# BinomialLLC/basis_universal

Measured on AMD Instinct MI355X. Metric: encoder Mpixels/s (ETC1S frontend hot path), higher is better.
Workload: dtype u8/int32; 1 GPU; 4096x4096 synthetic RGBA (SURVEY 8d recipe, seed 1234), ETC1S -q128 comp_level 1, basisu_frontend init+compress with tiles resident in HBM; blocks=1048576, max_endpoint_clusters=2416, max_selector_clusters=2731, final_endpoint_clusters=2413, final_selector_clusters=2277, images_in_flight_per_gpu=1, parallelism=1 x one image per GPU (no collective)

## Files before the change

### basis_universal_amd/csrc/api_etc1s.cpp

```cpp
#include <atomic>
#include <cstdlib>
#include "api_internal.h"
#include "etc1s_kernels.h"
#include "mipmap_kernels.h"
#include "unique_kernels.h"
#include "bookkeeping_kernels.h"
#include "kmeans_kernels.h"
#include "host/seam_translate.h"

namespace {
constexpr uint32_t UP_PIECE_BLOCKS = 65536;
constexpr uint32_t UP_SLOTS = 8, UP_EVENTS = 64;
unsigned upload_threads() {
    static const unsigned t = [] {
        unsigned want = 4;
        if (const char* e = std::getenv("BU_UPLOAD_THREADS")) { const int v = std::atoi(e); if (v >= 1 && v <= 16) want = (unsigned)v; }
        const unsigned hw = std::thread::hardware_concurrency();
        return hw ? std::min(want, std::max(1u, hw / 2)) : 1u;
    }();
    return t;
}
}

extern "C" {

int bu_hip_set_pixel_blocks(bu_hip_context* ctx, size_t total_blocks, const bu_pixel_block* blocks) {
    if (!ctx) return 0;
    if (total_blocks > 0xFFFFFFFFull) { set_error(ctx, "too many blocks"); return 0; }
    device_guard g(ctx->device);
    BU_TRY(ctx, ctx->pixel_arena.reserve(total_blocks * sizeof(bu_pixel_block)));
    if (total_blocks) BU_TRY(ctx, h2d(ctx, ctx->pixel_arena.p, blocks, total_blocks * sizeof(bu_pixel_block)));
    BU_TRY(ctx, stream_wait(ctx, ctx->stream));
    ctx->d_pixel_blocks = ctx->pixel_arena.p;
    ctx->total_blocks = total_blocks;
    return 1;
}

int bu_hip_set_pixel_blocks_device(bu_hip_context* ctx, size_t total_blocks, const void* d_blocks) {
    if (!ctx || total_blocks > 0xFFFFFFFFull) return 0;
    ctx->d_pixel_blocks = d_blocks;
    ctx->total_blocks = total_blocks;
    return 1;
}

const void* bu_hip_get_pixel_blocks_device(const bu_hip_context* ctx, size_t* total_blocks) {
    if (!ctx) return nullptr;
    if (total_blocks) *total_blocks = ctx->total_blocks;
    return ctx->d_pixel_blocks;
}


int bu_hip_k_encode_etc1s_blocks(bu_hip_context* ctx, const void* d_px, uint32_t n, int quality, int perceptual, void* d_out) {
    if (!ctx) return 0;
    device_guard g(ctx->device);
    prof_scope ps(ctx, "encode_etc1s_blocks");
    BU_TRY(ctx, bu::launch_encode_etc1s_blocks(ctx->stream, d_px, n, quality, perceptual != 0, d_out));
    return 1;
}

int bu_hip_k_upload_and_encode_etc1s_blocks(bu_hip_context* ctx, void* d_px, const void* h_px, uint32_t n, int quality, int perceptual, void* d_out) {
    if (!ctx) return 0;
    if (!n) return 1;
    if (!d_px || !h_px || !d_out) { set_error(ctx, "upload_and_encode_etc1s_blocks: null argument"); return 0; }
    device_guard g(ctx->device);
    const uint32_t n_pieces = (n + UP_PIECE_BLOCKS - 1) / UP_PIECE_BLOCKS;
    if (ctx->wait_hook || n_pieces < 2 || !ensure_side_stream(ctx)) {
        BU_TRY(ctx, h2d(ctx, d_px, h_px, (size_t)n * 64));
        prof_scope ps(ctx, "encode_etc1s_blocks");
        BU_TRY(ctx, bu::launch_encode_etc1s_blocks(ctx->stream, d_px, n, quality, perceptual != 0, d_out));
        return 1;
    }
    while (ctx->up_events.size() < UP_EVENTS) {
        hipEvent_t e = nullptr;
        BU_TRY(ctx, hipEventCreateWithFlags(&e, hipEventDisableTiming));
        ctx->up_events.push_back(e);
    }
    bool pinned_src = false;
    {
        hipPointerAttribute_t a;
        if (hipPointerGetAttributes(&a, h_px) == hipSuccess) pinned_src = a.type == hipMemoryTypeHost;
        else (void)hipGetLastError();
    }
    const size_t piece_bytes = (size_t)UP_PIECE_BLOCKS * 64;
    if (!pinned_src && ctx->up_ring_cap < piece_bytes * UP_SLOTS) {
        if (ctx->up_ring) { (void)hipHostFree(ctx->up_ring); ctx->up_ring = nullptr; ctx->up_ring_cap = 0; }
        BU_TRY(ctx, hipHostMalloc(&ctx->up_ring, piece_bytes * UP_SLOTS, hipHostMallocDefault));
        ctx->up_ring_cap = piece_bytes * UP_SLOTS;
    }
    BU_TRY(ctx, hipEventRecord(ctx->side_fork, ctx->stream));
    BU_TRY(ctx, hipStreamWaitEvent(ctx->side_stream, ctx->side_fork, 0));
    const char* src = static_cast<const char*>(h_px);
    char* dst = static_cast<char*>(d_px);
    char* out = static_cast<char*>(d_out);
    std::vector<std::atomic<int>> ready(pinned_src ? 0 : n_pieces), issued(pinned_src ? 0 : n_pieces);
    std::atomic<int> stop{0};
    std::vector<std::thread> helpers;
    if (!pinned_src) {
        for (auto& r : ready) r.store(0, std::memory_order_relaxed);
        for (auto& r : issued) r.store(0, std::memory_order_relaxed);
        const unsigned T = std::min<unsigned>(upload_threads(), n_pieces);
        try {
            for (unsigned t = 0; t < T; t++)
                helpers.emplace_back([&, t, T] {
                    (void)hipSetDevice(ctx->device);
                    for (uint32_t i = t; i < n_pieces && !stop.load(std::memory_order_acquire); i += T) {
                        if (i >= UP_SLOTS) {
                            while (!issued[i - UP_SLOTS].load(std::memory_order_acquire)) { if (stop.load(std::memory_order_acquire)) return; std::this_thread::yield(); }
                            (void)hipEventSynchronize(ctx->up_events[(i - UP_SLOTS) % UP_EVENTS]);
                        }
                        const size_t at = (size_t)i * piece_bytes, bytes = std::min(piece_bytes, (size_t)n * 64 - at);
                        std::memcpy(static_cast<char*>(ctx->up_ring) + (size_t)(i % UP_SLOTS) * piece_bytes, src + at, bytes);
                        ready[i].store(1, std::memory_order_release);
                    }
                });
        } catch (...) {
            stop.store(1); for (auto& h : helpers) h.join();
            set_error(ctx, "upload_and_encode_etc1s_blocks: could not start the helper threads");
            return 0;
        }
    }
    hipError_t err = hipSuccess;
    {
        prof_scope ps(ctx, "upload_and_encode_etc1s_blocks");
        for (uint32_t i = 0; i < n_pieces && err == hipSuccess; i++) {
            const size_t at = (size_t)i * piece_bytes, bytes = std::min(piece_bytes, (size_t)n * 64 - at);
            const uint32_t blocks = (uint32_t)(bytes / 64);
            const void* from = src + at;
            if (!pinned_src) {
                while (!ready[i].load(std::memory_order_acquire)) std::this_thread::yield();
                from = static_cast<char*>(ctx->up_ring) + (size_t)(i % UP_SLOTS) * piece_bytes;
            }
            hipEvent_t ev = ctx->up_events[i % UP_EVENTS];
            if ((err = hipMemcpyAsync(dst + at, from, bytes, hipMemcpyHostToDevice, ctx->side_stream)) != hipSuccess) break;
            if ((err = hipEventRecord(ev, ctx->side_stream)) != hipSuccess) break;
            if (!pinned_src) issued[i].store(1, std::memory_order_release);
            if ((err = hipStreamWaitEvent(ctx->stream, ev, 0)) != hipSuccess) break;
            err = bu::launch_encode_etc1s_blocks(ctx->stream, dst + at, blocks, quality, perceptual != 0, out + (size_t)i * UP_PIECE_BLOCKS * 8);
        }
    }
    if (err != hipSuccess) stop.store(1, std::memory_order_release);
    for (auto& h : helpers) h.join();
    const hipError_t drained = hipStreamSynchronize(ctx->side_stream);
    if (err == hipSuccess) err = drained;
    if (err != hipSuccess) { set_error(ctx, "upload_and_encode_etc1s_blocks: %s", hipGetErrorString(err)); return 0; }
    return 1;
}

int bu_hip_k_endpoint_training_vectors(bu_hip_context* ctx, const void* d_etc, uint32_t n, float* d_out6) {
    if (!ctx) return 0;
    device_guard g(ctx->device);
    prof_scope ps(ctx, "endpoint_training_vectors");
    BU_TRY(ctx, bu::launch_endpoint_training_vectors(ctx->stream, d_etc, n, d_out6));
    return 1;
}

static int codebook_fit_split(bu_hip_context* ctx, const std::vector<uint32_t>& order, const uint32_t* h_offsets, const void* d_px, const void* d_enc, const uint32_t* d_offsets,
                              const uint32_t* d_indices, int quality, bool perceptual, bool forced, uint32_t step, uint8_t* d_params, uint64_t* d_err, uint8_t* d_valid,
                              uint64_t* d_cur_err, const char* label) {
    const uint32_t wide_min = ctx->tuning.codebook_wide_min;
    std::vector<uint32_t> small_ones, big_cluster, big_first, big_sub;
    for (uint32_t c : order) {
        const uint32_t sub = h_offsets[c + 1] - h_offsets[c];
        if (wide_min && sub && (uint64_t)sub * 8u >= wide_min && sub < (1u << 28)) { big_cluster.push_back(c); big_first.push_back(h_offsets[c]); big_sub.push_back(sub); }
        else small_ones.push_back(c);
    }
    std::vector<unsigned char> image;
    bu::cb_wide_layout L{};
    if (!big_cluster.empty()) L = bu::codebook_wide_prepare(big_cluster.data(), big_first.data(), big_sub.data(), (uint32_t)big_cluster.size(), image);
    arena& ord = ctx->scratch[5];
    const size_t ord_bytes = (small_ones.size() * sizeof(uint32_t) + 255) & ~(size_t)255;
    BU_TRY(ctx, ord.reserve(ord_bytes + L.total));
    char* work = static_cast<char*>(ord.p) + ord_bytes;
    if (!small_ones.empty()) BU_TRY(ctx, h2d(ctx, ord.p, small_ones.data(), small_ones.size() * sizeof(uint32_t)));
    if (!image.empty()) BU_TRY(ctx, h2d(ctx, work, image.data(), image.size()));
    {
        prof_scope ps(ctx, label);
        if (!small_ones.empty()) {
            if (forced) BU_TRY(ctx, bu::launch_refit_endpoints_given_selectors(ctx->stream, d_px, d_enc, (uint32_t)small_ones.size(), static_cast<const uint32_t*>(ord.p), d_offsets, d_indices,
                                                                               quality, perceptual, d_params, d_err, d_valid, d_cur_err));
            else BU_TRY(ctx, bu::launch_generate_endpoint_codebook(ctx->stream, d_px, (uint32_t)small_ones.size(), static_cast<const uint32_t*>(ord.p), d_offsets, d_indices,
                                                                   quality, perceptual, step, d_params, d_err, d_valid));
        }
        if (L.n_big) BU_TRY(ctx, bu::launch_codebook_wide(ctx->stream, d_px, d_indices, work, L, quality, perceptual, forced, step, d_enc, d_params, d_err, d_valid, d_cur_err));
    }
    return 1;
}

int bu_hip_k_cluster_colour_means(bu_hip_context* ctx, const void* d_px, uint32_t n_clusters, const uint32_t* h_offsets, const uint32_t* d_indices, float* h_out) {
    if (!ctx) return 0;
    if (!n_clusters) return 1;
    if (!d_px || !h_offsets || !d_indices || !h_out) { set_error(ctx, "cluster_colour_means: null argument"); return 0; }
    device_guard g(ctx->device);
    std::vector<uint32_t> cl(n_clusters), first(n_clusters), sub(n_clusters);
    for (uint32_t c = 0; c < n_clusters; c++) {
        cl[c] = c; first[c] = h_offsets[c]; sub[c] = h_offsets[c + 1] - h_offsets[c];
        if (!sub[c]) { set_error(ctx, "cluster_colour_means: empty cluster %u", c); return 0; }
    }
    std::vector<unsigned char> image;
    const bu::cb_wide_layout L = bu::codebook_wide_prepare(cl.data(), first.data(), sub.data(), n_clusters, image);
    arena& ws = ctx->scratch[5];
    const size_t out_at = (L.total + 255) & ~(size_t)255;
    BU_TRY(ctx, ws.reserve(out_at + (size_t)n_clusters * 12));
    BU_TRY(ctx, h2d(ctx, ws.p, image.data(), image.size()));
    float* d_out = reinterpret_cast<float*>(static_cast<char*>(ws.p) + out_at);
    BU_TRY(ctx, bu::launch_codebook_wide_means(ctx->stream, d_px, d_indices, ws.p, L, d_out));
    if (!fetch(ctx, h_out, d_out, (size_t)n_clusters * 12)) return 0;
    return 1;
}

static std::vector<uint32_t> size_descending_order(const uint32_t* h_offsets, uint32_t n) {
    std::vector<uint32_t> order(n), tmp(n), key(n);
    uint32_t largest = 0;
    for (uint32_t i = 0; i < n; i++) largest = std::max(largest, h_offsets[i + 1] - h_offsets[i]);
    for (uint32_t i = 0; i < n; i++) { order[i] = i; key[i] = largest - (h_offsets[i + 1] - h_offsets[i]); }
    for (uint32_t shift = 0; shift < 32 && (largest >> shift); shift += 11) {
        uint32_t count[2049] = {};
        for (uint32_t i = 0; i < n; i++) count[((key[order[i]] >> shift) & 2047u) + 1]++;
        for (uint32_t b = 0; b < 2048; b++) count[b + 1] += count[b];
        for (uint32_t i = 0; i < n; i++) tmp[count[(key[order[i]] >> shift) & 2047u]++] = order[i];
        order.swap(tmp);
    }
    return order;
}

int bu_hip_k_generate_endpoint_codebook_part(bu_hip_context* ctx, const void* d_px, uint32_t n_clusters, const uint32_t* h_offsets,
                                             const uint32_t* d_offsets, const uint32_t* d_indices, int quality, int perceptual, uint32_t step,
                                             uint8_t* d_params, uint64_t* d_err, uint8_t* d_valid, uint32_t part, uint32_t parts) {
    if (!ctx) return 0;
    if (!n_clusters) return 1;
    if (!parts || part >= parts) { set_error(ctx, "generate_endpoint_codebook: bad part %u of %u", part, parts); return 0; }
    device_guard g(ctx->device);
    const std::vector<uint32_t> order = size_descending_order(h_offsets, n_clusters);
    std::vector<uint32_t> mine;
    for (uint32_t i = part; i < n_clusters; i += parts) mine.push_back(order[i]);
    if (mine.empty()) return 1;
    return codebook_fit_split(ctx, mine, h_offsets, d_px, nullptr, d_offsets, d_indices, quality, perceptual != 0, false, step, d_params, d_err, d_valid, nullptr, "generate_endpoint_codebook");
}

int bu_hip_k_generate_endpoint_codebook(bu_hip_context* ctx, const void* d_px, uint32_t n_clusters, const uint32_t* h_offsets,
                                        const uint32_t* d_offsets, const uint32_t* d_indices, int quality, int perceptual, uint32_t step,
                                        uint8_t* d_params, uint64_t* d_err, uint8_t* d_valid) {
    return bu_hip_k_generate_endpoint_codebook_part(ctx, d_px, n_clusters, h_offsets, d_offsets, d_indices, quality, perceptual, step, d_params, d_err, d_valid, 0, 1);
}

int bu_hip_k_refit_endpoints_given_selectors_q(bu_hip_context* ctx, const void* d_px, const void* d_enc, uint32_t n_clusters, const uint32_t* h_offsets,
                                               const uint32_t* d_offsets, const uint32_t* d_indices, int quality, int perceptual, uint8_t* d_params, uint64_t* d_err,
                                             uint8_t* d_valid, uint64_t* d_cur_err) {
    if (!ctx) return 0;
    if (!n_clusters) return 1;
    device_guard g(ctx->device);
    const std::vector<uint32_t> order = size_descending_order(h_offsets, n_clusters);
    return codebook_fit_split(ctx, order, h_offsets, d_px, d_enc, d_offsets, d_indices, quality == BU_ETC_QUALITY_SLOW ? BU_ETC_QUALITY_SLOW : BU_ETC_QUALITY_UBER, perceptual != 0, true, 0u,
                              d_params, d_err, d_valid, d_cur_err, "refit_endpoints_given_selectors");
}

int bu_hip_k_refit_endpoints_given_selectors(bu_hip_context* ctx, const void* d_px, const void* d_enc, uint32_t n_clusters, const uint32_t* h_offsets,
                                             const uint32_t* d_offsets, const uint32_t* d_indices, int perceptual, uint8_t* d_params, uint64_t* d_err,
                                             uint8_t* d_valid, uint64_t* d_cur_err) {
    return bu_hip_k_refit_endpoints_given_selectors_q(ctx, d_px, d_enc, n_clusters, h_offsets, d_offsets, d_indices, BU_ETC_QUALITY_UBER, perceptual, d_params, d_err, d_valid, d_cur_err);
}

int bu_hip_k_subblock_errors(bu_hip_context* ctx, const void* d_px, uint32_t n_blocks, const uint32_t* d_block_cluster, const uint8_t* d_cluster_params,
                             int perceptual, uint64_t* d_out) {
    if (!ctx) return 0;
    device_guard g(ctx->device);
    prof_scope ps(ctx, "subblock_errors");
    BU_TRY(ctx, bu::launch_subblock_errors(ctx->stream, d_px, n_blocks, d_block_cluster, d_cluster_params, perceptual != 0, d_out));
    return 1;
}

int bu_hip_k_backend_block_errors(bu_hip_context* ctx, const void* d_px, const void* d_etc_blocks, const uint32_t* d_block_cluster, const uint8_t* d_cluster_params,
                                  uint32_t first_block, uint32_t num_blocks_x, uint32_t num_blocks_y, uint32_t n_clusters, int perceptual, int with_neighbours,
                                  uint32_t* d_own_err, uint32_t* d_neighbour_err) {
    if (!ctx) return 0;
    if (!d_px || !d_etc_blocks || !d_block_cluster || !d_cluster_params || !d_own_err || (with_neighbours && !d_neighbour_err)) { set_error(ctx, "backend_block_errors: null argument"); return 0; }
    device_guard g(ctx->device);
    prof_scope ps(ctx, "backend_block_errors");
    BU_TRY(ctx, bu::launch_backend_block_errors(ctx->stream, d_px, d_etc_blocks, d_block_cluster, d_cluster_params, first_block, num_blocks_x, num_blocks_y, n_clusters, perceptual != 0,
                                                with_neighbours != 0, d_own_err, d_neighbour_err));
    return 1;
}

int bu_hip_k_refine_endpoint_clusterization(bu_hip_context* ctx, const void* d_px, uint32_t n_blocks, const uint32_t* d_block_cluster,
                                            const uint8_t* d_cluster_params, uint32_t n_clusters, uint32_t n_parents, const uint32_t* d_cand_offsets,
                                            const uint32_t* d_cand_indices, const uint8_t* d_block_parent, int perceptual, uint32_t* d_out_best) {
    if (!ctx) return 0;
    device_guard g(ctx->device);
    void* work = nullptr;
    if (const size_t wb = ctx->tuning.refine_unsorted ? 0 : bu::refine_workspace_bytes(n_clusters, n_parents)) { BU_TRY(ctx, ctx->refine_lists.reserve(wb)); work = ctx->refine_lists.p; }
    prof_scope ps(ctx, "refine_endpoint_clusterization");
    BU_TRY(ctx, bu::launch_refine_endpoint_clusterization(ctx->stream, d_px, n_blocks, d_block_cluster, d_cluster_params, n_clusters, n_parents,
                                                          d_cand_offsets, d_cand_indices, d_block_parent, perceptual != 0, d_out_best, work));
    return 1;
}

int bu_hip_k_extract_blocks(bu_hip_context* ctx, const void* d_rgba, uint32_t width, uint32_t height, uint32_t pitch_bytes, void* d_out) {
    if (!ctx) return 0;
    if (!d_rgba || !d_out || !width || !height || pitch_bytes < width * 4u) { set_error(ctx, "extract_blocks: bad arguments"); return 0; }
    device_guard g(ctx->device);
    prof_scope ps(ctx, "extract_blocks");
    BU_TRY(ctx, bu::launch_extract_blocks(ctx->stream, d_rgba, width, height, pitch_bytes, d_out));
    return 1;
}

int bu_hip_k_extract_slices(bu_hip_context* ctx, const bu_hip_slice_source* slices, uint32_t n, void* d_out) {
    if (!ctx) return 0;
    static const char* const fn = "extract_slices";
    static_assert(sizeof(bu_hip_slice_source) == 32, "the kernel reads a record as two 16-byte words");
    if (!n) { set_error(ctx, "%s: no slices (n == 0)", fn); return 0; }
    if (!slices || !d_out) { set_error(ctx, "%s: null pointer", fn); return 0; }
    if ((uintptr_t)d_out & 15u) { set_error(ctx, "%s: the output is not 16-byte aligned", fn); return 0; }
    const size_t table_at = (size_t)n * sizeof(bu_hip_slice_source), bytes = table_at + ((size_t)n + 1) * sizeof(uint32_t);
    std::vector<uint8_t> pack(bytes);
    uint32_t* prefix = reinterpret_cast<uint32_t*>(pack.data() + table_at);
    uint64_t total = 0, end = 0;
    for (uint32_t i = 0; i < n; i++) {
        const bu_hip_slice_source& s = slices[i];
        if (!s.d_raster) { set_error(ctx, "%s: slice %u: null raster", fn, i); return 0; }
        if (!s.width || !s.height) { set_error(ctx, "%s: slice %u: zero size (%u x %u)", fn, i, s.width, s.height); return 0; }
        if (s.width > 0x7fffffffu || s.height > 0x7fffffffu) { set_error(ctx, "%s: slice %u: %u x %u pixels is too large", fn, i, s.width, s.height); return 0; }
        if ((uint64_t)s.pitch_bytes < (uint64_t)s.width * 4u) { set_error(ctx, "%s: slice %u: row pitch %u bytes is less than 4 * width = %llu", fn, i, s.pitch_bytes, (unsigned long long)s.width * 4u); return 0; }
        if (s.mode > BU_HIP_SLICE_ALPHA) { set_error(ctx, "%s: slice %u: unknown mode %u", fn, i, s.mode); return 0; }
        if (s.first_block < end) { set_error(ctx, "%s: slice %u: first_block %llu lies before the end of slice %u's blocks (%llu): ranges must ascend without overlap", fn, i, (unsigned long long)s.first_block, i ? i - 1 : 0, (unsigned long long)end); return 0; }
        const uint64_t tiles = (((uint64_t)s.width + 3u) / 4u) * (((uint64_t)s.height + 3u) / 4u);
        prefix[i] = (uint32_t)total;
        total += tiles;
        if (tiles > ((uint64_t)1 << 30) || total > ((uint64_t)1 << 30)) { set_error(ctx, "%s: more than 2^30 tiles in one call (at slice %u)", fn, i); return 0; }
        end = s.first_block + tiles;
    }
    prefix[n] = (uint32_t)total;
    std::memcpy(pack.data(), slices, table_at);
    device_guard g(ctx->device);
    arena& table = ctx->scratch[4];
    BU_TRY(ctx, table.reserve(bytes));
    BU_TRY(ctx, h2d(ctx, table.p, pack.data(), bytes));
    prof_scope ps(ctx, fn);
    BU_TRY(ctx, bu::launch_extract_slices(ctx->stream, static_cast<const bu_hip_slice_source*>(table.p), reinterpret_cast<const uint32_t*>(static_cast<const uint8_t*>(table.p) + table_at),
                                          n, (uint32_t)total, d_out));
    return 1;
}

int bu_hip_k_resample_rgba8(bu_hip_context* ctx, const void* d_src, uint32_t src_w, uint32_t src_h, void* d_dst, uint32_t dst_w, uint32_t dst_h,
                            const uint32_t* x_first, const uint16_t* x_pixel, const float* x_weight, const uint32_t* y_first, const uint16_t* y_pixel, const float* y_weight,
                            int x_after_y, int srgb, const float* srgb_to_linear, const uint8_t* linear_to_srgb, uint32_t num_comps) {
    if (!ctx) return 0;
    if (!d_src || !d_dst || !src_w || !src_h || !dst_w || !dst_h || !x_first || !x_pixel || !x_weight || !y_first || !y_pixel || !y_weight || !srgb_to_linear ||
        !linear_to_srgb || num_comps < 3 || num_comps > 4 || src_w > 16384 || src_h > 16384) { set_error(ctx, "resample_rgba8: bad arguments"); return 0; }
    device_guard g(ctx->device);
    const size_t nx = x_first[dst_w], ny = y_first[dst_h];
    for (uint32_t i = 0; i < nx; i++) if (x_pixel[i] >= src_w) { set_error(ctx, "resample_rgba8: x contributor out of range"); return 0; }
    for (uint32_t i = 0; i < ny; i++) if (y_pixel[i] >= src_h) { set_error(ctx, "resample_rgba8: y contributor out of range"); return 0; }
    auto pad = [](size_t v) { return (v + 15) & ~(size_t)15; };
    const size_t o_xf = 0, o_xw = pad(o_xf + (dst_w + 1) * 4), o_xp = pad(o_xw + nx * 4), o_yf = pad(o_xp + nx * 2), o_yw = pad(o_yf + (dst_h + 1) * 4), o_yp = pad(o_yw + ny * 4),
                 o_t0 = pad(o_yp + ny * 2), o_t1 = o_t0 + 1024, total = o_t1 + 8192;
    std::vector<uint8_t> pack(total, 0);
    std::memcpy(&pack[o_xf], x_first, (dst_w + 1) * 4); std::memcpy(&pack[o_xw], x_weight, nx * 4); std::memcpy(&pack[o_xp], x_pixel, nx * 2);
    std::memcpy(&pack[o_yf], y_first, (dst_h + 1) * 4); std::memcpy(&pack[o_yw], y_weight, ny * 4); std::memcpy(&pack[o_yp], y_pixel, ny * 2);
    std::memcpy(&pack[o_t0], srgb_to_linear, 1024); std::memcpy(&pack[o_t1], linear_to_srgb, 8192);
    arena &lists = ctx->scratch[4], &tmp = ctx->scratch[5];
    const size_t tmp_px = std::max((size_t)dst_w * src_h, (size_t)src_w * dst_h);
    BU_TRY(ctx, lists.reserve(total));
    BU_TRY(ctx, tmp.reserve(tmp_px * 16));
    BU_TRY(ctx, h2d(ctx, lists.p, pack.data(), total));
    const char* b = static_cast<const char*>(lists.p);
    {
        prof_scope ps(ctx, "resample_rgba8");
        BU_TRY(ctx, bu::launch_resample_rgba8(ctx->stream, d_src, src_w, src_h, d_dst, dst_w, dst_h, (const uint32_t*)(b + o_xf), (const uint16_t*)(b + o_xp), (const float*)(b + o_xw),
                                              (const uint32_t*)(b + o_yf), (const uint16_t*)(b + o_yp), (const float*)(b + o_yw), x_after_y != 0, srgb != 0,
                                              (const float*)(b + o_t0), (const uint8_t*)(b + o_t1), num_comps, tmp.p));
    }
    BU_TRY(ctx, stream_wait(ctx, ctx->stream));
    return 1;
}

int bu_hip_k_determine_selectors(bu_hip_context* ctx, const void* d_px, uint32_t n_blocks, const uint8_t* d_color5_inten,
                                 const uint32_t* d_block_cluster, int perceptual, void* d_out) {
    if (!ctx) return 0;
    device_guard g(ctx->device);
    prof_scope ps(ctx, "determine_selectors");
    BU_TRY(ctx, bu::launch_determine_selectors(ctx->stream, d_px, n_blocks, d_color5_inten, d_block_cluster, perceptual != 0, d_out));
    return 1;
}

int bu_hip_k_selector_training_vectors(bu_hip_context* ctx, const void* d_enc, uint32_t n_blocks, int perceptual, float* d_out16, uint64_t* d_w) {
    if (!ctx) return 0;
    device_guard g(ctx->device);
    prof_scope ps(ctx, "selector_training_vectors");
    BU_TRY(ctx, bu::launch_selector_training_vectors(ctx->stream, d_enc, n_blocks, perceptual != 0, d_out16, d_w));
    return 1;
}

int bu_hip_k_create_optimized_selector_codebook(bu_hip_context* ctx, const void* d_px, const void* d_enc, uint32_t n_clusters,
                                                const uint32_t* d_offsets, const uint32_t* d_block_indices, int perceptual, void* d_selector_blocks) {
    if (!ctx) return 0;
    device_guard g(ctx->device);
    if (!n_clusters) return 1;
    arena& ws = ctx->scratch[4];
    BU_TRY(ctx, ws.reserve(bu::create_optimized_selector_codebook_workspace_bytes(n_clusters)));
    prof_scope ps(ctx, "create_optimized_selector_codebook");
    BU_TRY(ctx, bu::launch_create_optimized_selector_codebook(ctx->stream, d_px, d_enc, n_clusters, d_offsets, d_block_indices, perceptual != 0, ws.p,
                                                              d_selector_blocks));
    return 1;
}

int bu_hip_k_find_optimal_selector_clusters(bu_hip_context* ctx, const void* d_px, void* d_enc, uint32_t n_blocks, const void* d_selector_blocks,
                                            uint32_t n_selectors, uint32_t n_parents, const uint32_t* d_cand_offsets, const uint32_t* d_cand_indices,
                                            const uint8_t* d_block_parent, int perceptual, uint32_t chunk, uint32_t* d_out) {
    if (!ctx) return 0;
    device_guard g(ctx->device);
    prof_scope ps(ctx, "find_optimal_selector_clusters");
    arena& tmp = ctx->scratch[4];
    const size_t idx_bytes = ((size_t)n_blocks * sizeof(uint32_t) + 255) & ~(size_t)255;
    size_t words = (size_t)(n_parents ? n_parents : 1u) * n_selectors;
    if (words * 4 > ((size_t)64 << 20)) words = 0;
    BU_TRY(ctx, tmp.reserve(idx_bytes + words * 4));
    BU_TRY(ctx, bu::launch_find_optimal_selector_clusters(ctx->stream, d_px, d_enc, n_blocks, d_selector_blocks, n_selectors, n_parents, d_cand_offsets,
                                                          d_cand_indices, d_block_parent, perceptual != 0, chunk, static_cast<uint32_t*>(tmp.p), d_out,
                                                          words ? reinterpret_cast<uint32_t*>(static_cast<char*>(tmp.p) + idx_bytes) : nullptr, words));
    return 1;
}


int bu_hip_k_map_blocks_from_groups(bu_hip_context* ctx, const uint32_t* d_goffs, const uint32_t* d_idx, uint32_t n, uint32_t u_total, const uint32_t* d_leaf,
                                    const uint32_t* d_first_pos, const uint32_t* d_parent_of_unique, uint32_t* d_cluster, uint32_t* d_pos, uint8_t* d_parent) {
    if (!ctx) return 0;
    if (n && (!d_goffs || !d_idx || !d_leaf || !d_cluster || (d_pos && !d_first_pos))) { set_error(ctx, "map_blocks_from_groups: null pointer"); return 0; }
    device_guard g(ctx->device);
    prof_scope ps(ctx, "map_blocks_from_groups");
    BU_TRY(ctx, bu::launch_blocks_from_groups(ctx->stream, d_goffs, d_idx, n, u_total, d_leaf, d_first_pos, d_parent_of_unique, d_cluster, d_pos, d_parent));
    return 1;
}

int bu_hip_k_map_rank_blocks(bu_hip_context* ctx, const uint32_t* d_cluster, uint32_t n, uint32_t k, uint32_t* d_sizes, uint32_t* d_offsets, uint32_t* d_sorted, uint32_t* d_pos) {
    if (!ctx) return 0;
    if (n && (!d_cluster || !d_sizes || !d_offsets || !d_sorted)) { set_error(ctx, "map_rank_blocks: null pointer"); return 0; }
    device_guard g(ctx->device);
    arena& ws = ctx->scratch[4];
    BU_TRY(ctx, ws.reserve(bu::rank_blocks_workspace_bytes(n, k)));
    prof_scope ps(ctx, "map_rank_blocks");
    BU_TRY(ctx, bu::launch_rank_blocks(ctx->stream, d_cluster, n, k, ws.p, d_sizes, d_offsets, d_sorted, d_pos));
    return 1;
}

int bu_hip_k_map_endpoint_csr(bu_hip_context* ctx, const uint32_t* d_cluster, const uint32_t* d_pos, uint32_t n, const uint32_t* d_offsets, uint32_t* d_indices) {
    if (!ctx) return 0;
    device_guard g(ctx->device);
    prof_scope ps(ctx, "map_endpoint_csr");
    BU_TRY(ctx, bu::launch_endpoint_csr_fill(ctx->stream, d_cluster, d_pos, n, d_offsets, d_indices));
    return 1;
}

int bu_hip_k_map_remap(bu_hip_context* ctx, uint32_t* d_cluster, uint32_t* d_pos, uint32_t n, const uint32_t* d_new_index, const uint32_t* d_base) {
    if (!ctx) return 0;
    device_guard g(ctx->device);
    prof_scope ps(ctx, "map_remap");
    BU_TRY(ctx, bu::launch_remap_clusters(ctx->stream, d_cluster, d_pos, n, d_new_index, d_base));
    return 1;
}

int bu_hip_k_map_count_differences(bu_hip_context* ctx, const uint32_t* d_a, const uint32_t* d_b, uint32_t n, uint32_t* d_count) {
    if (!ctx) return 0;
    device_guard g(ctx->device);
    BU_TRY(ctx, bu::launch_count_differences(ctx->stream, d_a, d_b, n, d_count));
    return 1;
}

int bu_hip_k_map_membership(bu_hip_context* ctx, const uint8_t* d_parent, const uint32_t* d_cluster, uint32_t n, uint32_t parents, uint32_t clusters, uint8_t* d_flags) {
    if (!ctx) return 0;
    device_guard g(ctx->device);
    BU_TRY(ctx, bu::launch_membership(ctx->stream, d_parent, d_cluster, n, parents, clusters, d_flags));
    return 1;
}

int bu_hip_k_map_gather(bu_hip_context* ctx, const uint32_t* d_table, const uint32_t* d_index, uint32_t n, uint32_t* d_out) {
    if (!ctx) return 0;
    device_guard g(ctx->device);
    BU_TRY(ctx, bu::launch_gather_u32(ctx->stream, d_table, d_index, n, d_out));
    return 1;
}


int bu_hip_kmeans_codebook(bu_hip_context* ctx, int kind, const void* d_keys, const uint64_t* d_weights, const uint32_t* d_goffs, uint32_t n, uint32_t max_clusters,
                           uint32_t n_parents, uint32_t iterations, uint32_t* d_cluster, uint32_t* d_parent, uint32_t* out_clusters, uint32_t* out_parents) {
    if (!ctx) return 0;
    if (!d_keys || !d_cluster || !out_clusters || !n || !max_clusters || (kind == 0 && !d_weights) || (kind != 0 && !d_goffs) || (n_parents && !d_parent)) {
        set_error(ctx, "kmeans_codebook: bad arguments");
        return 0;
    }
    device_guard g(ctx->device);
    const uint32_t k = std::min(max_clusters, n);
    arena& ws = ctx->scratch[3];
    BU_TRY(ctx, ws.reserve(bu::kmeans_workspace_bytes(n, k) + (size_t)k * 8 + 256));
    const bu::kmeans_buffers b = bu::kmeans_carve(ws.p, n, k);
    uint32_t* d_tab = reinterpret_cast<uint32_t*>(static_cast<char*>(ws.p) + bu::kmeans_workspace_bytes(n, k));
    {
        prof_scope ps(ctx, kind ? "kmeans_endpoints" : "kmeans_selectors");
        BU_TRY(ctx, bu::launch_kmeans(ctx->stream, kind, d_keys, d_weights, d_goffs, n, k, iterations, b, d_cluster));
    }
    std::vector<uint64_t> sums((size_t)k * 17);
    std::vector<float> cen((size_t)k * 16);
    {
        mail_fetch f(ctx);
        BU_TRY(ctx, f.add(sums.data(), b.sums, sums.size() * 8));
        BU_TRY(ctx, f.add(cen.data(), b.cen, cen.size() * 4));
        if (!f.wait()) return 0;
    }
    std::vector<uint32_t> old_to_new(k, 0), live;
    for (uint32_t c = 0; c < k; c++) if (sums[(size_t)c * 17 + 16]) { old_to_new[c] = (uint32_t)live.size(); live.push_back(c); }
    const uint32_t kl = (uint32_t)live.size();
    *out_clusters = kl;
    uint32_t parents = 0;
    std::vector<uint32_t> parent_of_old(k, 0);
    if (n_parents && kl) {
        const int D = 16;
        std::vector<double> pts((size_t)kl * D), wts(kl);
        for (uint32_t i = 0; i < kl; i++) {
            const uint64_t w = sums[(size_t)live[i] * 17 + 16];
            wts[i] = (double)w;
            for (int d = 0; d < D; d++) pts[(size_t)i * D + d] = (double)sums[(size_t)live[i] * 17 + d] / (double)w;
        }
        const uint32_t P = std::min(n_parents, kl);
        std::vector<double> pc((size_t)P * D);
        for (uint32_t p = 0; p < P; p++) std::memcpy(&pc[(size_t)p * D], &pts[(size_t)(((uint64_t)p * 2 + 1) * kl / (2ull * P)) * D], D * sizeof(double));
        std::vector<uint32_t> owner(kl, 0);
        for (int it = 0; it < 12; it++) {
            for (uint32_t i = 0; i < kl; i++) {
                double bd = 1e300; uint32_t bp = 0;
                for (uint32_t p = 0; p < P; p++) {
                    double dd = 0;
                    for (int d = 0; d < D; d++) { const double t = pts[(size_t)i * D + d] - pc[(size_t)p * D + d]; dd += t * t; }
                    if (dd < bd) { bd = dd; bp = p; }
                }
                owner[i] = bp;
            }
            std::vector<double> acc((size_t)P * D, 0.0), aw(P, 0.0);
            for (uint32_t i = 0; i < kl; i++) { aw[owner[i]] += wts[i]; for (int d = 0; d < D; d++) acc[(size_t)owner[i] * D + d] += wts[i] * pts[(size_t)i * D + d]; }
            for (uint32_t p = 0; p < P; p++) if (aw[p] > 0) for (int d = 0; d < D; d++) pc[(size_t)p * D + d] = acc[(size_t)p * D + d] / aw[p];
        }
        std::vector<int32_t> renum(P, -1);
        for (uint32_t i = 0; i < kl; i++) if (renum[owner[i]] < 0) renum[owner[i]] = 0;
        for (uint32_t p = 0; p < P; p++) if (renum[p] == 0) renum[p] = (int32_t)parents++;
        for (uint32_t i = 0; i < kl; i++) parent_of_old[live[i]] = (uint32_t)renum[owner[i]];
    }
    if (out_parents) *out_parents = parents;
    if (n_parents) {
        BU_TRY(ctx, h2d(ctx, d_tab, parent_of_old.data(), (size_t)k * 4));
        BU_TRY(ctx, bu::launch_gather_u32(ctx->stream, d_tab, d_cluster, n, d_parent));
    }
    BU_TRY(ctx, h2d(ctx, d_tab + k, old_to_new.data(), (size_t)k * 4));
    BU_TRY(ctx, bu::launch_gather_u32(ctx->stream, d_tab + k, d_cluster, n, d_cluster));
    BU_TRY(ctx, stream_wait(ctx, ctx->stream));
    (void)cen;
    return 1;
}

int bu_hip_k_kmeans_seed(bu_hip_context* ctx, int kind, const void* d_keys, const uint64_t* d_weights, const uint32_t* d_goffs, uint32_t n, uint32_t k, uint32_t* d_pick,
                         float* d_centroids) {
    if (!ctx) return 0;
    if (!d_keys || !d_pick || !d_centroids || !n || !k || k > n || (kind == 0 && !d_weights) || (kind != 0 && !d_goffs)) {
        set_error(ctx, "kmeans_seed: bad arguments");
        return 0;
    }
    device_guard g(ctx->device);
    arena& ws = ctx->scratch[3];
    BU_TRY(ctx, ws.reserve(bu::kmeans_workspace_bytes(n, k)));
    const bu::kmeans_buffers b = bu::kmeans_carve(ws.p, n, k);
    const uint64_t* weights = nullptr;
    BU_TRY(ctx, bu::kmeans_begin(ctx->stream, kind, d_keys, d_weights, d_goffs, n, b, &weights));
    bu::kmeans_seed(ctx->stream, n, k, b);
    BU_TRY(ctx, hipGetLastError());
    BU_TRY(ctx, hipMemcpyAsync(d_pick, b.pick, (size_t)k * 4, hipMemcpyDeviceToDevice, ctx->stream));
    BU_TRY(ctx, hipMemcpyAsync(d_centroids, b.cen, (size_t)k * 16 * 4, hipMemcpyDeviceToDevice, ctx->stream));
    return 1;
}

int bu_hip_k_kmeans_round(bu_hip_context* ctx, int kind, const void* d_keys, const uint64_t* d_weights, const uint32_t* d_goffs, uint32_t n, uint32_t k, float* d_centroids,
                          uint64_t* d_live, int update, uint32_t* d_assign, uint64_t* d_sums, uint64_t* d_worst) {
    if (!ctx) return 0;
    if (!d_keys || !d_centroids || !d_assign || !d_sums || !n || !k || k > n || (kind == 0 && !d_weights) || (kind != 0 && !d_goffs) || (update && !d_live)) {
        set_error(ctx, "kmeans_round: bad arguments");
        return 0;
    }
    device_guard g(ctx->device);
    arena& ws = ctx->scratch[3];
    BU_TRY(ctx, ws.reserve(bu::kmeans_workspace_bytes(n, k)));
    const bu::kmeans_buffers b = bu::kmeans_carve(ws.p, n, k);
    hipStream_t st = ctx->stream;
    const uint64_t* weights = nullptr;
    BU_TRY(ctx, bu::kmeans_begin(st, kind, d_keys, d_weights, d_goffs, n, b, &weights));
    bu::kmeans_flags(st, kind, n, k, b);
    BU_TRY(ctx, hipMemcpyAsync(b.cen, d_centroids, (size_t)k * 16 * 4, hipMemcpyDeviceToDevice, st));
    if (d_live) bu::kmeans_set_live(st, d_live, k, b);
    BU_TRY(ctx, bu::kmeans_assign_round(st, kind, weights, n, k, b, d_live != nullptr, update || d_worst, d_assign, 0));
    BU_TRY(ctx, hipMemcpyAsync(d_sums, b.sums, (size_t)k * 17 * 8, hipMemcpyDeviceToDevice, st));
    if (d_worst) BU_TRY(ctx, hipMemcpyAsync(d_worst, bu::kmeans_wg_worst(b), (size_t)bu::kmeans_workgroups(n) * 8, hipMemcpyDeviceToDevice, st));
    if (update) {
        BU_TRY(ctx, bu::kmeans_update_round(st, n, k, b));
        BU_TRY(ctx, hipMemcpyAsync(d_centroids, b.cen, (size_t)k * 16 * 4, hipMemcpyDeviceToDevice, st));
        bu::kmeans_get_live(st, d_live, k, b);
    }
    BU_TRY(ctx, hipGetLastError());
    return 1;
}

int bu_hip_k_unique_endpoint_vectors(bu_hip_context* ctx, const void* d_etc1_blocks, uint32_t n_blocks, uint32_t* d_sorted_block_idx, uint64_t* d_unique_keys,
                                     uint32_t* d_group_offsets, uint32_t* out_unique) {
    if (!ctx) return 0;
    if (!out_unique || (n_blocks && (!d_etc1_blocks || !d_sorted_block_idx || !d_unique_keys || !d_group_offsets))) { set_error(ctx, "unique_endpoint_vectors: null pointer"); return 0; }
    *out_unique = 0;
    if (!n_blocks) return 1;
    device_guard g(ctx->device);
    arena& ws = ctx->scratch[4];
    BU_TRY(ctx, ws.reserve(bu::unique_endpoint_vectors_workspace_bytes(n_blocks)));
    uint32_t* d_n = nullptr;
    {
        prof_scope ps(ctx, "unique_endpoint_vectors");
        BU_TRY(ctx, bu::launch_unique_endpoint_vectors(ctx->stream, d_etc1_blocks, n_blocks, ws.p, d_sorted_block_idx, d_unique_keys, d_group_offsets, &d_n));
    }
    if (!fetch(ctx, out_unique, d_n, 4)) return 0;
    return 1;
}

int bu_hip_k_unique_selector_vectors(bu_hip_context* ctx, const void* d_enc_blocks, const uint64_t* d_weights, uint32_t n_blocks, uint32_t* d_sorted_block_idx,
                                     uint32_t* d_unique_keys, uint64_t* d_unique_weights, uint32_t* d_group_offsets, uint32_t* out_unique) {
    if (!ctx) return 0;
    if (!out_unique || (n_blocks && (!d_enc_blocks || !d_weights || !d_sorted_block_idx || !d_unique_keys || !d_unique_weights || !d_group_offsets))) {
        set_error(ctx, "unique_selector_vectors: null pointer");
        return 0;
    }
    *out_unique = 0;
    if (!n_blocks) return 1;
    device_guard g(ctx->device);
    arena& ws = ctx->scratch[4];
    BU_TRY(ctx, ws.reserve(bu::unique_selector_vectors_workspace_bytes(n_blocks)));
    uint32_t* d_n = nullptr;
    {
        prof_scope ps(ctx, "unique_selector_vectors");
        BU_TRY(ctx, bu::launch_unique_selector_vectors(ctx->stream, d_enc_blocks, d_weights, n_blocks, ws.p, d_sorted_block_idx, d_unique_keys, d_unique_weights,
                                                        d_group_offsets, &d_n));
    }
    if (!fetch(ctx, out_unique, d_n, 4)) return 0;
    return 1;
}


int bu_hip_encode_etc1s_blocks(bu_hip_context* ctx, bu_etc_block* out, int perceptual, uint32_t total_perms) {
    if (!ctx || !ctx->d_pixel_blocks) { if (ctx) set_error(ctx, "no pixel blocks set"); return 0; }
    device_guard g(ctx->device);
    const uint32_t n = (uint32_t)ctx->total_blocks;
    arena& o = ctx->scratch[0];
    BU_TRY(ctx, o.reserve((size_t)n * 8));
    BU_TRY(ctx, bu::launch_encode_etc1s_blocks(ctx->stream, ctx->d_pixel_blocks, n, quality_from_perms(total_perms), perceptual != 0, o.p));
    if (!fetch(ctx, out, o.p, (size_t)n * 8)) return 0;
    return 1;
}

int bu_hip_determine_selectors(bu_hip_context* ctx, const bu_color_rgba* color5_inten, bu_etc_block* out, int perceptual) {
    if (!ctx || !ctx->d_pixel_blocks) { if (ctx) set_error(ctx, "no pixel blocks set"); return 0; }
    device_guard g(ctx->device);
    const uint32_t n = (uint32_t)ctx->total_blocks;
    arena &in = ctx->scratch[0], &o = ctx->scratch[1];
    BU_TRY(ctx, in.reserve((size_t)n * 4));
    BU_TRY(ctx, o.reserve((size_t)n * 8));
    BU_TRY(ctx, h2d(ctx, in.p, color5_inten, (size_t)n * 4));
    BU_TRY(ctx, bu::launch_determine_selectors(ctx->stream, ctx->d_pixel_blocks, n, static_cast<const uint8_t*>(in.p), nullptr, perceptual != 0, o.p));
    if (!fetch(ctx, out, o.p, (size_t)n * 8)) return 0;
    return 1;
}

int bu_hip_refine_endpoint_clusterization(bu_hip_context* ctx, const bu_block_info* info, uint32_t total_clusters, const bu_endpoint_cluster* clusters,
                                          const uint32_t* , uint32_t* out, int perceptual) {
    if (!ctx || !ctx->d_pixel_blocks) { if (ctx) set_error(ctx, "no pixel blocks set"); return 0; }
    device_guard g(ctx->device);
    const uint32_t n = (uint32_t)ctx->total_blocks;
    if (n && !out) { set_error(ctx, "refine: null pointer"); return 0; }
    bu::seam::refine_tables t;
    if (const char* e = bu::seam::translate_refine(info, n, total_clusters, clusters, t)) { set_error(ctx, "%s", e); return 0; }
    if (!n) return 1;
    const uint32_t n_parents = t.win.n_parents();

    arena &a_par = ctx->scratch[0], &a_cur = ctx->scratch[1], &a_off = ctx->scratch[2], &a_idx = ctx->scratch[3], &a_out = ctx->scratch[4];
    arena& a_bp = ctx->scratch[5];
    BU_TRY(ctx, a_par.reserve(total_clusters * 4ull)); BU_TRY(ctx, a_cur.reserve(n * 4ull)); BU_TRY(ctx, a_off.reserve(t.win.cand_offsets.size() * 4ull));
    BU_TRY(ctx, a_idx.reserve(t.win.cand_indices.size() * 4ull + 4)); BU_TRY(ctx, a_out.reserve(n * 4ull)); BU_TRY(ctx, a_bp.reserve(n));
    BU_TRY(ctx, h2d(ctx, a_par.p, t.params.data(), total_clusters * 4ull));
    BU_TRY(ctx, h2d(ctx, a_cur.p, t.block_cur.data(), n * 4ull));
    BU_TRY(ctx, h2d(ctx, a_off.p, t.win.cand_offsets.data(), t.win.cand_offsets.size() * 4ull));
    BU_TRY(ctx, h2d(ctx, a_idx.p, t.win.cand_indices.data(), t.win.cand_indices.size() * 4ull));
    BU_TRY(ctx, h2d(ctx, a_bp.p, t.win.block_parent.data(), n));
    void* work = nullptr;
    if (const size_t wb = ctx->tuning.refine_unsorted ? 0 : bu::refine_workspace_bytes(total_clusters, n_parents)) { BU_TRY(ctx, ctx->refine_lists.reserve(wb)); work = ctx->refine_lists.p; }
    BU_TRY(ctx, bu::launch_refine_endpoint_clusterization(ctx->stream, ctx->d_pixel_blocks, n, static_cast<const uint32_t*>(a_cur.p),
                                                          static_cast<const uint8_t*>(a_par.p), total_clusters, n_parents,
                                                          static_cast<const uint32_t*>(a_off.p), static_cast<const uint32_t*>(a_idx.p),
                                                          static_cast<const uint8_t*>(a_bp.p), perceptual != 0, static_cast<uint32_t*>(a_out.p), work));
    std::vector<uint32_t> pos(n);
    if (!fetch(ctx, pos.data(), a_out.p, n * 4ull)) return 0;
    for (uint32_t b = 0; b < n; b++) out[b] = clusters[pos[b]].m_cluster_index;
    return 1;
}

int bu_hip_find_optimal_selector_clusters_for_each_block(bu_hip_context* ctx, const bu_fosc_block* info, uint32_t total_input_selectors,
                                                         const bu_fosc_selector* selectors, const uint32_t* selector_cluster_indices, uint32_t* out, int perceptual) {
    if (!ctx || !ctx->d_pixel_blocks) { if (ctx) set_error(ctx, "no pixel blocks set"); return 0; }
    device_guard g(ctx->device);
    const uint32_t n = (uint32_t)ctx->total_blocks;
    if (n && (!out || !selector_cluster_indices)) { set_error(ctx, "fosc: null pointer"); return 0; }
    bu::seam::fosc_tables t;
    if (const char* e = bu::seam::translate_fosc(info, n, total_input_selectors, selectors, t)) { set_error(ctx, "%s", e); return 0; }
    if (!n) return 1;
    const uint32_t n_parents = t.win.n_parents();

    arena &a_sel = ctx->scratch[0], &a_enc = ctx->scratch[1], &a_off = ctx->scratch[2], &a_idx = ctx->scratch[3], &a_tmp = ctx->scratch[4], &a_bp = ctx->scratch[5];
    BU_TRY(ctx, a_sel.reserve(total_input_selectors * 8ull + 8)); BU_TRY(ctx, a_enc.reserve(n * 8ull + n * 4ull)); BU_TRY(ctx, a_off.reserve(t.win.cand_offsets.size() * 4ull));
    BU_TRY(ctx, a_idx.reserve(t.win.cand_indices.size() * 4ull + 4)); BU_TRY(ctx, a_tmp.reserve(n * 4ull)); BU_TRY(ctx, a_bp.reserve(n));
    uint32_t* d_out = reinterpret_cast<uint32_t*>(static_cast<uint8_t*>(a_enc.p) + n * 8ull);
    BU_TRY(ctx, h2d(ctx, a_sel.p, t.selector_blocks.data(), total_input_selectors * 8ull));
    BU_TRY(ctx, h2d(ctx, a_enc.p, t.encoded_blocks.data(), n * 8ull));
    BU_TRY(ctx, h2d(ctx, a_off.p, t.win.cand_offsets.data(), t.win.cand_offsets.size() * 4ull));
    BU_TRY(ctx, h2d(ctx, a_idx.p, t.win.cand_indices.data(), t.win.cand_indices.size() * 4ull));
    BU_TRY(ctx, h2d(ctx, a_bp.p, t.win.block_parent.data(), n));
    BU_TRY(ctx, bu::launch_find_optimal_selector_clusters(ctx->stream, ctx->d_pixel_blocks, a_enc.p, n, a_sel.p, total_input_selectors, n_parents,
                                                          static_cast<const uint32_t*>(a_off.p), static_cast<const uint32_t*>(a_idx.p), static_cast<const uint8_t*>(a_bp.p),
                                                          perceptual != 0, 0, static_cast<uint32_t*>(a_tmp.p), d_out, nullptr, 0));
    std::vector<uint32_t> pos(n);
    if (!fetch(ctx, pos.data(), d_out, n * 4ull)) return 0;
    for (uint32_t b = 0; b < n; b++) out[b] = selector_cluster_indices[pos[b]];
    return 1;
}

int bu_hip_encode_etc1s_pixel_clusters(bu_hip_context* ctx, bu_etc_block* out, uint32_t total_clusters, const bu_pixel_cluster* clusters,
                                       uint64_t total_pixels, const bu_color_rgba* pixels, const uint32_t* weights, int perceptual, uint32_t total_perms) {
    if (!ctx) return 0;
    device_guard g(ctx->device);
    if (!total_clusters) return 1;
    if (!out) { set_error(ctx, "pixel clusters: null pointer"); return 0; }
    bu::seam::pixel_tables t;
    if (const char* e = bu::seam::translate_pixel_clusters(total_clusters, clusters, total_pixels, pixels, weights, t)) { set_error(ctx, "%s", e); return 0; }
    arena &a_px = ctx->scratch[0], &a_off = ctx->scratch[1], &a_idx = ctx->scratch[2], &a_par = ctx->scratch[3];
    const size_t params_bytes = ((total_clusters * 4ull + 7) / 8) * 8;
    BU_TRY(ctx, a_px.reserve(t.texels.size() * 4ull)); BU_TRY(ctx, a_off.reserve(t.offsets.size() * 4ull)); BU_TRY(ctx, a_idx.reserve(t.indices.size() * 4ull + 4));
    BU_TRY(ctx, a_par.reserve(params_bytes + total_clusters * 8ull + total_clusters));
    BU_TRY(ctx, h2d(ctx, a_px.p, t.texels.data(), t.texels.size() * 4ull));
    BU_TRY(ctx, h2d(ctx, a_off.p, t.offsets.data(), t.offsets.size() * 4ull));
    BU_TRY(ctx, h2d(ctx, a_idx.p, t.indices.data(), t.indices.size() * 4ull));
    uint8_t* d_params = static_cast<uint8_t*>(a_par.p);
    uint64_t* d_err = reinterpret_cast<uint64_t*>(d_params + params_bytes);
    uint8_t* d_valid = reinterpret_cast<uint8_t*>(d_err + total_clusters);
    if (!bu_hip_k_generate_endpoint_codebook(ctx, a_px.p, total_clusters, t.offsets.data(), static_cast<const uint32_t*>(a_off.p), static_cast<const uint32_t*>(a_idx.p),
                                             std::max(quality_from_perms(total_perms), (int)bu::BU_Q_MEDIUM), perceptual, 0, d_params, d_err, d_valid))
        return 0;
    std::vector<uint8_t> params(total_clusters * 4ull);
    if (!fetch(ctx, params.data(), d_params, params.size())) return 0;
    for (uint32_t c = 0; c < total_clusters; c++) {
        const uint64_t m = bu::seam::color5_inten_to_etc_block(params[c * 4], params[c * 4 + 1], params[c * 4 + 2], params[c * 4 + 3]);
        memcpy(&out[c], &m, 8);
    }
    return 1;
}
}
```

### basis_universal_amd/csrc/bookkeeping_kernels.hip

```cpp
#include <hip/hip_runtime.h>
#include <hipcub/hipcub.hpp>
#include <stdint.h>
#include <algorithm>

#include "bookkeeping_kernels.h"
#include "sort_pairs.h"
#include "tsvq_bufs.h"

namespace bu {

namespace {

__global__ void __launch_bounds__(256) k_blocks_from_groups(const uint32_t* __restrict__ goffs, const uint32_t* __restrict__ idx, uint32_t n, uint32_t u_total,
                                                            const uint32_t* __restrict__ leaf_of_unique, const uint32_t* __restrict__ first_pos,
                                                            const uint32_t* __restrict__ parent_of_unique, uint32_t* __restrict__ cluster, uint32_t* __restrict__ pos,
                                                            uint8_t* __restrict__ parent) {
    const uint32_t j = blockIdx.x * 256 + threadIdx.x;
    if (j >= n) return;
    uint32_t lo = 0, hi = u_total;
    while (hi - lo > 1) { const uint32_t mid = (lo + hi) >> 1; if (goffs[mid] <= j) lo = mid; else hi = mid; }
    const uint32_t u = lo, b = idx[j];
    cluster[b] = leaf_of_unique[u];
    if (pos) pos[b] = first_pos[u] + (j - goffs[u]);
    if (parent) parent[b] = parent_of_unique ? (uint8_t)parent_of_unique[u] : 0;
}

__global__ void __launch_bounds__(256) k_iota_copy(const uint32_t* __restrict__ src, uint32_t n, uint32_t* __restrict__ keys, uint32_t* __restrict__ vals) {
    const uint32_t i = blockIdx.x * 256 + threadIdx.x;
    if (i < n) { keys[i] = src[i]; vals[i] = i; }
}
__global__ void __launch_bounds__(256) k_offsets_from_sorted(const uint32_t* __restrict__ keys_sorted, uint32_t n, uint32_t k, uint32_t* __restrict__ offsets) {
    const uint32_t c = blockIdx.x * 256 + threadIdx.x;
    if (c > k) return;
    uint32_t lo = 0, hi = n;
    while (lo < hi) { const uint32_t mid = (lo + hi) >> 1; if (keys_sorted[mid] < c) lo = mid + 1; else hi = mid; }
    offsets[c] = lo;
}
__global__ void __launch_bounds__(256) k_sizes_from_offsets(const uint32_t* __restrict__ offsets, uint32_t k, uint32_t* __restrict__ sizes) {
    const uint32_t c = blockIdx.x * 256 + threadIdx.x;
    if (c <= k) sizes[c] = c < k ? offsets[c + 1] - offsets[c] : 0u;
}
__global__ void __launch_bounds__(256) k_positions(const uint32_t* __restrict__ keys_sorted, const uint32_t* __restrict__ blocks_sorted, uint32_t n,
                                                   const uint32_t* __restrict__ offsets, uint32_t* __restrict__ pos) {
    const uint32_t i = blockIdx.x * 256 + threadIdx.x;
    if (i < n) pos[blocks_sorted[i]] = i - offsets[keys_sorted[i]];
}

__global__ void __launch_bounds__(256) k_endpoint_csr_fill(const uint32_t* __restrict__ cluster, const uint32_t* __restrict__ pos, uint32_t n,
                                                           const uint32_t* __restrict__ offsets, uint32_t* __restrict__ indices) {
    const uint32_t b = blockIdx.x * 256 + threadIdx.x;
    if (b >= n) return;
    const size_t at = (size_t)offsets[cluster[b]] + 2ull * pos[b];
    indices[at] = b * 2; indices[at + 1] = b * 2 + 1;
}

__global__ void __launch_bounds__(256) k_remap_clusters(uint32_t* __restrict__ cluster, uint32_t* __restrict__ pos, uint32_t n, const uint32_t* __restrict__ new_index,
                                                        const uint32_t* __restrict__ base) {
    const uint32_t b = blockIdx.x * 256 + threadIdx.x;
    if (b >= n) return;
    const uint32_t old = cluster[b];
    if (pos && base) pos[b] += base[old];
    cluster[b] = new_index[old];
}

__global__ void __launch_bounds__(256) k_count_differences(const uint32_t* __restrict__ a, const uint32_t* __restrict__ b, uint32_t n, uint32_t* __restrict__ out) {
    __shared__ uint32_t s_c[4];
    uint32_t c = 0;
    for (uint32_t i = blockIdx.x * 256 + threadIdx.x; i < n; i += gridDim.x * 256) c += a[i] != b[i];
#pragma unroll
    for (int o = 32; o >= 1; o >>= 1) c += (uint32_t)__shfl_xor((int)c, o, 64);
    if ((threadIdx.x & 63) == 0) s_c[threadIdx.x >> 6] = c;
    __syncthreads();
    if (threadIdx.x == 0 && (s_c[0] | s_c[1] | s_c[2] | s_c[3])) atomicAdd(out, s_c[0] + s_c[1] + s_c[2] + s_c[3]);
}

__global__ void __launch_bounds__(256) k_membership(const uint8_t* __restrict__ parent, const uint32_t* __restrict__ cluster, uint32_t n, uint32_t clusters,
                                                    uint8_t* __restrict__ flags) {
    const uint32_t b = blockIdx.x * 256 + threadIdx.x;
    if (b < n) flags[(size_t)(parent ? parent[b] : 0) * clusters + cluster[b]] = 1;
}

__global__ void __launch_bounds__(256) k_scatter_spans(const uint32_t* __restrict__ perm0, const uint32_t* __restrict__ perm1, const bk_span* __restrict__ spans,
                                                       uint32_t* __restrict__ out) {
    const bk_span s = spans[blockIdx.x];
    const uint32_t* p = tsvq_list(perm0, perm1, s.buf) + s.start;
    for (uint32_t i = threadIdx.x; i < s.count; i += 256) out[p[i]] = s.value;
}

__global__ void __launch_bounds__(256) k_finish_spans(const uint32_t* __restrict__ perm0, const uint32_t* __restrict__ perm1, const bk_span* __restrict__ spans,
                                                      uint32_t* __restrict__ leaf_of, uint32_t* __restrict__ parent_of, const uint32_t* __restrict__ goffs,
                                                      uint32_t* __restrict__ first_pos, uint32_t* __restrict__ sizes) {
    __shared__ uint32_t s_wave[4];
    const bk_span s = spans[blockIdx.x];
    const uint32_t* p = tsvq_list(perm0, perm1, s.buf) + s.start;
    const int lane = threadIdx.x & 63, wave = threadIdx.x >> 6;
    uint32_t run = 0;
    for (uint32_t base = 0; base < s.count; base += 256) {
        const uint32_t i = base + threadIdx.x;
        const bool have = i < s.count;
        const uint32_t m = have ? p[i] : 0u;
        if (have) { leaf_of[m] = blockIdx.x; if (parent_of) parent_of[m] = s.value; }
        if (!goffs) continue;
        const uint32_t sz = have ? goffs[m + 1] - goffs[m] : 0u;
        uint32_t incl = sz;
#pragma unroll
        for (int o = 1; o < 64; o <<= 1) { const uint32_t t = (uint32_t)__shfl_up((int)incl, o, 64); if (lane >= o) incl += t; }
        __syncthreads();
        if (lane == 63) s_wave[wave] = incl;
        __syncthreads();
        uint32_t before = run;
        for (int w = 0; w < wave; w++) before += s_wave[w];
        if (have) first_pos[m] = before + incl - sz;
        run += s_wave[0] + s_wave[1] + s_wave[2] + s_wave[3];
    }
    if (goffs && threadIdx.x == 0) sizes[blockIdx.x] = run;
}

__global__ void __launch_bounds__(256) k_endpoint_rows(const uint64_t* __restrict__ keys, const uint32_t* __restrict__ goffs, uint32_t n, float* __restrict__ rows,
                                                       uint64_t* __restrict__ weights) {
    const uint32_t u = blockIdx.x * 256 + threadIdx.x;
    if (u >= n) return;
    const uint64_t k = keys[u];
#pragma unroll
    for (int c = 5; c >= 0; c--) rows[(size_t)u * 6 + (size_t)(5 - c)] = (float)(int)((k >> (8 * c)) & 255) * (1.0f / 255.0f);
    weights[u] = 2ull * (goffs[u + 1] - goffs[u]);
}

__global__ void __launch_bounds__(256) k_exchange_children(uint32_t* __restrict__ perm0, uint32_t* __restrict__ perm1, const bk_span* __restrict__ nodes ,
                                                           const uint8_t* __restrict__ take, uint32_t* __restrict__ staging, int dir) {
    const bk_span nd = nodes[blockIdx.x];
    uint32_t* child = tsvq_child_list(perm0, perm1, nd.buf) + nd.start;
    uint32_t* st = staging + nd.value;
    const bool mine = take[blockIdx.x] != 0;
    for (uint32_t i = threadIdx.x; i < nd.count; i += 256) {
        if (dir == 0) st[i] = mine ? child[i] : 0u;
        else if (mine) child[i] = st[i];
    }
}

__global__ void __launch_bounds__(256) k_gather_u32(const uint32_t* __restrict__ table, const uint32_t* index, uint32_t n, uint32_t* out) {
    const uint32_t i = blockIdx.x * 256 + threadIdx.x;
    if (i < n) out[i] = table[index[i]];
}

struct rank_temp { uint32_t *keys_in, *vals_in, *keys_sorted; void* cub; size_t cub_bytes; };

rank_temp carve_rank(void* ws, uint32_t n, uint32_t k, size_t* total) {
    auto up = [](size_t x) { return (x + 255) & ~(size_t)255; };
    size_t sort_bytes = 0, scan_bytes = 0;
    (void)sort_pairs<uint32_t, uint32_t>(nullptr, sort_bytes, nullptr, nullptr, nullptr, nullptr, n, 0, 32, nullptr);
    (void)hipcub::DeviceScan::ExclusiveSum(nullptr, scan_bytes, (const uint32_t*)nullptr, (uint32_t*)nullptr, (int)k + 1);
    rank_temp t;
    char* p = static_cast<char*>(ws);
    size_t off = 0;
    t.keys_in = reinterpret_cast<uint32_t*>(p + off); off += up((size_t)n * 4);
    t.vals_in = reinterpret_cast<uint32_t*>(p + off); off += up((size_t)n * 4);
    t.keys_sorted = reinterpret_cast<uint32_t*>(p + off); off += up((size_t)n * 4);
    t.cub = p + off; t.cub_bytes = up(sort_bytes > scan_bytes ? sort_bytes : scan_bytes); off += t.cub_bytes;
    if (total) *total = off;
    return t;
}

}

size_t rank_blocks_workspace_bytes(uint32_t n, uint32_t k) { size_t t = 0; carve_rank(nullptr, n ? n : 1, k, &t); return t; }

hipError_t launch_blocks_from_groups(hipStream_t st, const uint32_t* d_goffs, const uint32_t* d_idx, uint32_t n, uint32_t u_total, const uint32_t* d_leaf_of_unique,
                                     const uint32_t* d_first_pos, const uint32_t* d_parent_of_unique, uint32_t* d_cluster, uint32_t* d_pos, uint8_t* d_parent) {
    if (!n) return hipSuccess;
    hipLaunchKernelGGL(k_blocks_from_groups, dim3((n + 255) / 256), dim3(256), 0, st, d_goffs, d_idx, n, u_total, d_leaf_of_unique, d_first_pos, d_parent_of_unique, d_cluster,
                       d_pos, d_parent);
    return hipGetLastError();
}

hipError_t launch_rank_blocks(hipStream_t st, const uint32_t* d_cluster, uint32_t n, uint32_t k, void* d_ws, uint32_t* d_sizes, uint32_t* d_offsets,
                              uint32_t* d_sorted_blocks, uint32_t* d_pos) {
    if (!n) return hipSuccess;
    const rank_temp t = carve_rank(d_ws, n, k, nullptr);
    hipError_t e;
    const dim3 grid((n + 255) / 256), blk(256), gk((k + 256) / 256);
    hipLaunchKernelGGL(k_iota_copy, grid, blk, 0, st, d_cluster, n, t.keys_in, t.vals_in);
    int bits = 1;
    while (bits < 32 && (1u << bits) < k) bits++;
    size_t bytes = t.cub_bytes;
    if ((e = sort_pairs<uint32_t, uint32_t>(t.cub, bytes, t.keys_in, t.keys_sorted, t.vals_in, d_sorted_blocks, n, 0, (unsigned)bits, st)) != hipSuccess) return e;
    hipLaunchKernelGGL(k_offsets_from_sorted, gk, blk, 0, st, t.keys_sorted, n, k, d_offsets);
    hipLaunchKernelGGL(k_sizes_from_offsets, gk, blk, 0, st, d_offsets, k, d_sizes);
    if (d_pos) hipLaunchKernelGGL(k_positions, grid, blk, 0, st, t.keys_sorted, d_sorted_blocks, n, d_offsets, d_pos);
    return hipGetLastError();
}

hipError_t launch_endpoint_csr_fill(hipStream_t st, const uint32_t* d_cluster, const uint32_t* d_pos, uint32_t n, const uint32_t* d_offsets, uint32_t* d_indices) {
    if (!n) return hipSuccess;
    hipLaunchKernelGGL(k_endpoint_csr_fill, dim3((n + 255) / 256), dim3(256), 0, st, d_cluster, d_pos, n, d_offsets, d_indices);
    return hipGetLastError();
}

hipError_t launch_remap_clusters(hipStream_t st, uint32_t* d_cluster, uint32_t* d_pos, uint32_t n, const uint32_t* d_new_index, const uint32_t* d_base) {
    if (!n) return hipSuccess;
    hipLaunchKernelGGL(k_remap_clusters, dim3((n + 255) / 256), dim3(256), 0, st, d_cluster, d_pos, n, d_new_index, d_base);
    return hipGetLastError();
}

hipError_t launch_count_differences(hipStream_t st, const uint32_t* d_a, const uint32_t* d_b, uint32_t n, uint32_t* d_count) {
    hipError_t e = hipMemsetAsync(d_count, 0, 4, st);
    if (e != hipSuccess || !n) return e;
    hipLaunchKernelGGL(k_count_differences, dim3(std::min<uint32_t>((n + 255) / 256, 1024u)), dim3(256), 0, st, d_a, d_b, n, d_count);
    return hipGetLastError();
}

hipError_t launch_membership(hipStream_t st, const uint8_t* d_parent, const uint32_t* d_cluster, uint32_t n, uint32_t parents, uint32_t clusters, uint8_t* d_flags) {
    hipError_t e = hipMemsetAsync(d_flags, 0, (size_t)parents * clusters, st);
    if (e != hipSuccess || !n) return e;
    hipLaunchKernelGGL(k_membership, dim3((n + 255) / 256), dim3(256), 0, st, d_parent, d_cluster, n, clusters, d_flags);
    return hipGetLastError();
}

hipError_t launch_scatter_spans(hipStream_t st, const uint32_t* d_perm0, const uint32_t* d_perm1, const bk_span* d_spans, uint32_t n_spans, uint32_t* d_out) {
    if (!n_spans) return hipSuccess;
    hipLaunchKernelGGL(k_scatter_spans, dim3(n_spans), dim3(256), 0, st, d_perm0, d_perm1, d_spans, d_out);
    return hipGetLastError();
}

hipError_t launch_finish_spans(hipStream_t st, const uint32_t* d_perm0, const uint32_t* d_perm1, const bk_span* d_spans, uint32_t n_spans, uint32_t* d_leaf_of, uint32_t* d_parent_of,
                               const uint32_t* d_goffs, uint32_t* d_first_pos, uint32_t* d_sizes) {
    if (!n_spans) return hipSuccess;
    hipLaunchKernelGGL(k_finish_spans, dim3(n_spans), dim3(256), 0, st, d_perm0, d_perm1, d_spans, d_leaf_of, d_parent_of, d_goffs, d_first_pos, d_sizes);
    return hipGetLastError();
}

hipError_t launch_endpoint_rows(hipStream_t st, const uint64_t* d_keys, const uint32_t* d_goffs, uint32_t n, float* d_rows, uint64_t* d_weights) {
    if (!n) return hipSuccess;
    hipLaunchKernelGGL(k_endpoint_rows, dim3((n + 255) / 256), dim3(256), 0, st, d_keys, d_goffs, n, d_rows, d_weights);
    return hipGetLastError();
}

hipError_t launch_exchange_children(hipStream_t st, uint32_t* d_perm0, uint32_t* d_perm1, const bk_span* d_nodes, const uint8_t* d_take, uint32_t n_nodes, uint32_t* d_staging, int dir) {
    if (!n_nodes) return hipSuccess;
    hipLaunchKernelGGL(k_exchange_children, dim3(n_nodes), dim3(256), 0, st, d_perm0, d_perm1, d_nodes, d_take, d_staging, dir);
    return hipGetLastError();
}

hipError_t launch_gather_u32(hipStream_t st, const uint32_t* d_table, const uint32_t* d_index, uint32_t n, uint32_t* d_out) {
    if (!n) return hipSuccess;
    hipLaunchKernelGGL(k_gather_u32, dim3((n + 255) / 256), dim3(256), 0, st, d_table, d_index, n, d_out);
    return hipGetLastError();
}

}
```

### basis_universal_amd/csrc/sort_pairs.h

```cpp
#pragma once
#include <hip/hip_runtime.h>
#include <rocprim/rocprim.hpp>

namespace bu {

using sort_pairs_config = rocprim::radix_sort_config<rocprim::default_config, rocprim::default_config, rocprim::default_config, 32768>;

template <class Key, class Value>
inline hipError_t sort_pairs(void* temporary, size_t& bytes, const Key* keys_in, Key* keys_out, const Value* values_in, Value* values_out, size_t n, unsigned begin_bit, unsigned end_bit,
                             hipStream_t stream) {
    return rocprim::radix_sort_pairs<sort_pairs_config>(temporary, bytes, keys_in, keys_out, values_in, values_out, n, begin_bit, end_bit, stream);
}

}
```

### basis_universal_amd/csrc/unique_kernels.hip

```cpp
#include <hip/hip_runtime.h>
#include <hipcub/hipcub.hpp>
#include <stdint.h>

#include <algorithm>
#include <mutex>
#include <vector>

#include "unique_kernels.h"
#include "sort_pairs.h"

namespace bu {

namespace {

__global__ void __launch_bounds__(256) k_selector_keys(const uint64_t* __restrict__ enc_blocks, uint32_t n, uint32_t* __restrict__ keys, uint32_t* __restrict__ idx) {
    const uint32_t b = blockIdx.x * 256 + threadIdx.x;
    if (b >= n) return;
    const uint32_t lo = (uint32_t)__builtin_bswap64(enc_blocks[b]);
    uint32_t key = 0;
#pragma unroll
    for (uint32_t i = 0; i < 16; i++) {
        const uint32_t bit = (i & 3u) * 4u + (i >> 2);
        const uint32_t raw = ((lo >> bit) & 1u) | (((lo >> (16u + bit)) & 1u) << 1);
        key = (key << 2) | ((0x1Eu >> (raw * 2u)) & 3u);
    }
    keys[b] = key;
    idx[b] = b;
}

__global__ void __launch_bounds__(256) k_close_offsets(const uint32_t* __restrict__ n_runs, uint32_t n, uint32_t* __restrict__ offsets) {
    if (blockIdx.x == 0 && threadIdx.x == 0) offsets[*n_runs] = n;
}

__global__ void __launch_bounds__(256) k_gather_weights(const uint32_t* __restrict__ idx, const uint64_t* __restrict__ weights, uint32_t n, uint64_t* __restrict__ out) {
    const uint32_t j = blockIdx.x * 256 + threadIdx.x;
    if (j < n) out[j] = weights[idx[j]];
}

__host__ __device__ inline uint64_t endpoint_key_of_code(uint32_t code) {
    const int r5 = (int)((code >> 13) & 31), g5 = (int)((code >> 8) & 31), b5 = (int)((code >> 3) & 31), inten = (int)(code & 7);
    const int big[8] = { 8, 17, 29, 42, 60, 80, 106, 183 };
    const int d = big[inten];
    const int r = (r5 << 3) | (r5 >> 2), g = (g5 << 3) | (g5 >> 2), bl = (b5 << 3) | (b5 >> 2);
    auto c8 = [](int x) -> uint64_t { return (uint64_t)(x < 0 ? 0 : (x > 255 ? 255 : x)); };
    return (c8(r - d) << 40) | (c8(g - d) << 32) | (c8(bl - d) << 24) | (c8(r + d) << 16) | (c8(g + d) << 8) | c8(bl + d);
}
constexpr uint32_t ENDPOINT_CODES = 1u << 18;
struct endpoint_rank_tables { uint32_t* rank_of_code = nullptr; uint64_t* key_of_rank = nullptr; uint32_t n_ranks = 0; hipError_t status = hipErrorNotInitialized; };

const endpoint_rank_tables& endpoint_tables(int device) {
    static endpoint_rank_tables tables[64];
    static std::once_flag once[64];
    if (device < 0 || device >= 64) { static const endpoint_rank_tables bad; return bad; }
    std::call_once(once[device], [device] {
        endpoint_rank_tables& t = tables[device];
        std::vector<std::pair<uint64_t, uint32_t>> kc(ENDPOINT_CODES);
        for (uint32_t c = 0; c < ENDPOINT_CODES; c++) kc[c] = { endpoint_key_of_code(c), c };
        std::sort(kc.begin(), kc.end());
        std::vector<uint32_t> rank(ENDPOINT_CODES);
        std::vector<uint64_t> keys;
        keys.reserve(ENDPOINT_CODES);
        for (uint32_t i = 0; i < ENDPOINT_CODES; i++) {
            if (i == 0 || kc[i].first != kc[i - 1].first) keys.push_back(kc[i].first);
            rank[kc[i].second] = (uint32_t)keys.size() - 1;
        }
        t.n_ranks = (uint32_t)keys.size();
        hipError_t e = hipMalloc(reinterpret_cast<void**>(&t.rank_of_code), ENDPOINT_CODES * sizeof(uint32_t));
        if (e == hipSuccess) e = hipMalloc(reinterpret_cast<void**>(&t.key_of_rank), keys.size() * sizeof(uint64_t));
        if (e == hipSuccess) e = hipMemcpy(t.rank_of_code, rank.data(), ENDPOINT_CODES * sizeof(uint32_t), hipMemcpyHostToDevice);
        if (e == hipSuccess) e = hipMemcpy(t.key_of_rank, keys.data(), keys.size() * sizeof(uint64_t), hipMemcpyHostToDevice);
        t.status = e;
    });
    return tables[device];
}

__global__ void __launch_bounds__(256) k_endpoint_ranks(const uint64_t* __restrict__ etc1_blocks, uint32_t n, const uint32_t* __restrict__ rank_of_code,
                                                        uint32_t* __restrict__ ranks, uint32_t* __restrict__ idx) {
    const uint32_t b = blockIdx.x * 256 + threadIdx.x;
    if (b >= n) return;
    const uint64_t v = __builtin_bswap64(etc1_blocks[b]);
    const uint32_t code = (uint32_t)(((v >> 59) & 31) << 13 | ((v >> 51) & 31) << 8 | ((v >> 43) & 31) << 3 | ((v >> 37) & 7));
    ranks[b] = rank_of_code[code];
    idx[b] = b;
}
__global__ void __launch_bounds__(256) k_keys_of_ranks(const uint32_t* __restrict__ ranks, const uint32_t* __restrict__ n_runs, const uint64_t* __restrict__ key_of_rank,
                                                       uint32_t n, uint64_t* __restrict__ keys) {
    const uint32_t u = blockIdx.x * 256 + threadIdx.x;
    if (u < n && u < *n_runs) keys[u] = key_of_rank[ranks[u]];
}

struct unique_temp { uint32_t *keys_in, *idx_in, *keys_sorted, *counts, *n_runs, *keys_again; uint64_t* w_sorted; void* cub; size_t cub_bytes; };
size_t align_up(size_t v) { return (v + 255) & ~(size_t)255; }

size_t cub_bytes_for(uint32_t n) {
    size_t a = 0, b = 0, c = 0, d = 0;
    uint32_t* p = nullptr;
    uint64_t* w = nullptr;
    (void)sort_pairs<uint32_t, uint32_t>(nullptr, a, p, p, p, p, n, 0, 32, nullptr);
    (void)hipcub::DeviceRunLengthEncode::Encode(nullptr, b, p, p, p, p, (int)n);
    (void)hipcub::DeviceScan::ExclusiveSum(nullptr, c, p, p, (int)n);
    (void)hipcub::DeviceReduce::ReduceByKey(nullptr, d, p, p, w, w, p, hipcub::Sum(), (int)n);
    return std::max(std::max(a, b), std::max(c, d));
}

unique_temp carve(void* base, uint32_t n, size_t* total) {
    char* p = static_cast<char*>(base);
    size_t o = 0;
    unique_temp t;
    t.keys_in = reinterpret_cast<uint32_t*>(p + o); o += align_up((size_t)n * 4);
    t.idx_in = reinterpret_cast<uint32_t*>(p + o); o += align_up((size_t)n * 4);
    t.keys_sorted = reinterpret_cast<uint32_t*>(p + o); o += align_up((size_t)n * 4);
    t.counts = reinterpret_cast<uint32_t*>(p + o); o += align_up((size_t)n * 4);
    t.n_runs = reinterpret_cast<uint32_t*>(p + o); o += 256;
    t.keys_again = reinterpret_cast<uint32_t*>(p + o); o += align_up((size_t)n * 4);
    t.w_sorted = reinterpret_cast<uint64_t*>(p + o); o += align_up((size_t)n * 8);
    t.cub_bytes = cub_bytes_for(n);
    t.cub = p + o; o += align_up(t.cub_bytes);
    if (total) *total = o;
    return t;
}

struct unique64_temp { uint64_t *keys_in, *keys_sorted; uint32_t *idx_in, *counts, *n_runs; void* cub; size_t cub_bytes; };
size_t cub_bytes_for64(uint32_t n) {
    size_t a = 0, b = 0, c = 0;
    uint64_t* k = nullptr;
    uint32_t* p = nullptr;
    (void)sort_pairs<uint64_t, uint32_t>(nullptr, a, k, k, p, p, n, 0, 64, nullptr);
    (void)hipcub::DeviceRunLengthEncode::Encode(nullptr, b, k, k, p, p, (int)n);
    (void)hipcub::DeviceScan::ExclusiveSum(nullptr, c, p, p, (int)n);
    size_t a32 = 0, b32 = 0;
    (void)sort_pairs<uint32_t, uint32_t>(nullptr, a32, p, p, p, p, n, 0, 18, nullptr);
    (void)hipcub::DeviceRunLengthEncode::Encode(nullptr, b32, p, p, p, p, (int)n);
    return std::max(std::max(a, a32), std::max(std::max(b, b32), c));
}
unique64_temp carve64(void* base, uint32_t n, size_t* total) {
    char* p = static_cast<char*>(base);
    size_t o = 0;
    unique64_temp t;
    t.keys_in = reinterpret_cast<uint64_t*>(p + o); o += align_up((size_t)n * 8);
    t.keys_sorted = reinterpret_cast<uint64_t*>(p + o); o += align_up((size_t)n * 8);
    t.idx_in = reinterpret_cast<uint32_t*>(p + o); o += align_up((size_t)n * 4);
    t.counts = reinterpret_cast<uint32_t*>(p + o); o += align_up((size_t)n * 4);
    t.n_runs = reinterpret_cast<uint32_t*>(p + o); o += 256;
    t.cub_bytes = cub_bytes_for64(n);
    t.cub = p + o; o += align_up(t.cub_bytes);
    if (total) *total = o;
    return t;
}

}

size_t unique_endpoint_vectors_workspace_bytes(uint32_t n_blocks) {
    size_t total = 0;
    carve64(nullptr, n_blocks ? n_blocks : 1, &total);
    return total;
}

hipError_t launch_unique_endpoint_vectors(hipStream_t st, const void* d_etc1_blocks, uint32_t n, void* d_workspace, uint32_t* d_sorted_block_idx, uint64_t* d_unique_keys,
                                          uint32_t* d_group_offsets, uint32_t** d_n_unique) {
    const unique64_temp t = carve64(d_workspace, n, nullptr);
    if (d_n_unique) *d_n_unique = t.n_runs;
    if (!n) return hipMemsetAsync(t.n_runs, 0, 4, st);
    int device = 0;
    hipError_t e = hipGetDevice(&device);
    if (e != hipSuccess) return e;
    const endpoint_rank_tables& tab = endpoint_tables(device);
    if (tab.status != hipSuccess) return tab.status;
    uint32_t* ranks_in = reinterpret_cast<uint32_t*>(t.keys_in);
    uint32_t* ranks_sorted = ranks_in + n;
    uint32_t* ranks_unique = reinterpret_cast<uint32_t*>(t.keys_sorted);
    hipLaunchKernelGGL(k_endpoint_ranks, dim3((n + 255) / 256), dim3(256), 0, st, static_cast<const uint64_t*>(d_etc1_blocks), n, tab.rank_of_code, ranks_in, t.idx_in);
    size_t bytes = t.cub_bytes;
    e = sort_pairs<uint32_t, uint32_t>(t.cub, bytes, ranks_in, ranks_sorted, t.idx_in, d_sorted_block_idx, n, 0, 18, st);
    if (e != hipSuccess) return e;
    bytes = t.cub_bytes;
    e = hipcub::DeviceRunLengthEncode::Encode(t.cub, bytes, ranks_sorted, ranks_unique, t.counts, t.n_runs, (int)n, st);
    if (e != hipSuccess) return e;
    bytes = t.cub_bytes;
    e = hipcub::DeviceScan::ExclusiveSum(t.cub, bytes, t.counts, d_group_offsets, (int)n, st);
    if (e != hipSuccess) return e;
    hipLaunchKernelGGL(k_close_offsets, dim3(1), dim3(64), 0, st, t.n_runs, n, d_group_offsets);
    const uint32_t most = n < tab.n_ranks ? n : tab.n_ranks;
    hipLaunchKernelGGL(k_keys_of_ranks, dim3((most + 255) / 256), dim3(256), 0, st, ranks_unique, t.n_runs, tab.key_of_rank, most, d_unique_keys);
    return hipGetLastError();
}

size_t unique_selector_vectors_workspace_bytes(uint32_t n_blocks) {
    size_t total = 0;
    carve(nullptr, n_blocks ? n_blocks : 1, &total);
    return total;
}

hipError_t launch_unique_selector_vectors(hipStream_t st, const void* d_enc_blocks, const uint64_t* d_weights, uint32_t n, void* d_workspace, uint32_t* d_sorted_block_idx,
                                          uint32_t* d_unique_keys, uint64_t* d_unique_weights, uint32_t* d_group_offsets, uint32_t** d_n_unique) {
    const unique_temp t = carve(d_workspace, n, nullptr);
    if (d_n_unique) *d_n_unique = t.n_runs;
    if (!n) return hipMemsetAsync(t.n_runs, 0, 4, st);
    hipLaunchKernelGGL(k_selector_keys, dim3((n + 255) / 256), dim3(256), 0, st, static_cast<const uint64_t*>(d_enc_blocks), n, t.keys_in, t.idx_in);
    size_t bytes = t.cub_bytes;
    hipError_t e = sort_pairs<uint32_t, uint32_t>(t.cub, bytes, t.keys_in, t.keys_sorted, t.idx_in, d_sorted_block_idx, n, 0, 32, st);
    if (e != hipSuccess) return e;
    bytes = t.cub_bytes;
    e = hipcub::DeviceRunLengthEncode::Encode(t.cub, bytes, t.keys_sorted, d_unique_keys, t.counts, t.n_runs, (int)n, st);
    if (e != hipSuccess) return e;
    bytes = t.cub_bytes;
    e = hipcub::DeviceScan::ExclusiveSum(t.cub, bytes, t.counts, d_group_offsets, (int)n, st);
    if (e != hipSuccess) return e;
    hipLaunchKernelGGL(k_close_offsets, dim3(1), dim3(64), 0, st, t.n_runs, n, d_group_offsets);
    hipLaunchKernelGGL(k_gather_weights, dim3((n + 255) / 256), dim3(256), 0, st, d_sorted_block_idx, d_weights, n, t.w_sorted);
    bytes = t.cub_bytes;
    e = hipcub::DeviceReduce::ReduceByKey(t.cub, bytes, t.keys_sorted, t.keys_again, t.w_sorted, d_unique_weights, t.n_runs + 1, hipcub::Sum(), (int)n, st);
    if (e != hipSuccess) return e;
    return hipGetLastError();
}

}
```

### include/basisu_hip.h

```cpp
#ifndef BASISU_HIP_H
#define BASISU_HIP_H
#include <stddef.h>
#include <stdint.h>

#ifdef __cplusplus
extern "C" {
#endif

#if defined(__GNUC__)
#define BU_HIP_API __attribute__((visibility("default")))
#else
#define BU_HIP_API
#endif


typedef struct bu_hip_context bu_hip_context;

#pragma pack(push, 1)
typedef struct { uint8_t m_pixels[16][4]; } bu_pixel_block;
typedef struct { uint8_t m_bytes[8]; } bu_etc_block;
typedef struct { uint8_t r, g, b, a; } bu_color_rgba;
typedef struct { uint64_t m_total_pixels, m_first_pixel_index; } bu_pixel_cluster;
typedef struct { uint16_t m_first_cluster_ofs, m_num_clusters, m_cur_cluster_index; uint8_t m_cur_cluster_etc_inten; } bu_block_info;
typedef struct { bu_color_rgba m_unscaled_color; uint8_t m_etc_inten; uint16_t m_cluster_index; } bu_endpoint_cluster;
typedef struct { uint32_t m_packed_selectors; } bu_fosc_selector;
typedef struct { bu_color_rgba m_etc_color5_inten; uint32_t m_first_selector, m_num_selectors; } bu_fosc_block;
#pragma pack(pop)

#define BU_HIP_ENCODE_ETC1S_MAX_PERMS 165u

BU_HIP_API int  bu_hip_init(int force_serialization);
BU_HIP_API void bu_hip_deinit(void);
BU_HIP_API int  bu_hip_is_available(void);
BU_HIP_API bu_hip_context* bu_hip_create_context(void);
BU_HIP_API void bu_hip_destroy_context(bu_hip_context*);

BU_HIP_API int bu_hip_set_pixel_blocks(bu_hip_context*, size_t total_blocks, const bu_pixel_block* pixel_blocks);
BU_HIP_API int bu_hip_encode_etc1s_blocks(bu_hip_context*, bu_etc_block* output_blocks, int perceptual, uint32_t total_perms);
BU_HIP_API int bu_hip_encode_etc1s_pixel_clusters(bu_hip_context*, bu_etc_block* output_blocks, uint32_t total_clusters,
    const bu_pixel_cluster* clusters, uint64_t total_pixels, const bu_color_rgba* pixels, const uint32_t* pixel_weights,
    int perceptual, uint32_t total_perms);
BU_HIP_API int bu_hip_refine_endpoint_clusterization(bu_hip_context*, const bu_block_info* pixel_block_info, uint32_t total_clusters,
    const bu_endpoint_cluster* cluster_info, const uint32_t* sorted_block_indices, uint32_t* output_cluster_indices, int perceptual);
BU_HIP_API int bu_hip_find_optimal_selector_clusters_for_each_block(bu_hip_context*, const bu_fosc_block* input_block_info,
    uint32_t total_input_selectors, const bu_fosc_selector* input_selectors, const uint32_t* selector_cluster_indices,
    uint32_t* output_selector_cluster_indices, int perceptual);
BU_HIP_API int bu_hip_determine_selectors(bu_hip_context*, const bu_color_rgba* input_etc_color5_and_inten, bu_etc_block* output_blocks, int perceptual);

typedef struct { uint8_t m_bytes[16]; } bu_uastc_block;
BU_HIP_API int bu_hip_encode_uastc_blocks(bu_hip_context*, bu_uastc_block* output_blocks, uint32_t flags);


BU_HIP_API bu_hip_context* bu_hip_create_context_on(int device);
typedef void (*bu_hip_destroy_fn)(void* user);
BU_HIP_API int  bu_hip_on_destroy(bu_hip_context*, bu_hip_destroy_fn fn, void* user);
BU_HIP_API void bu_hip_cancel_on_destroy(bu_hip_context*, bu_hip_destroy_fn fn, void* user);
BU_HIP_API int   bu_hip_context_device(const bu_hip_context*);
BU_HIP_API int   bu_hip_set_stream(bu_hip_context*, void* hip_stream);
BU_HIP_API void* bu_hip_get_stream(bu_hip_context*);
BU_HIP_API int   bu_hip_sync(bu_hip_context*);
typedef struct bu_hip_tuning {
    uint32_t struct_bytes;
    uint32_t tsvq_wide_min;
    uint32_t tsvq_wide6_min;
    uint32_t tsvq_wide_cov_min;
    uint32_t tsvq_windows;
    uint32_t tsvq_dense_min;
    uint32_t tsvq_zero_copy;
    uint32_t tsvq_chained_only;
    uint32_t tsvq_poll;
    uint32_t refine_unsorted;
    uint32_t debug;
    uint32_t tsvq_deep_levels;
    uint32_t uastc_walk_cus;
    uint32_t codebook_wide_min;
} bu_hip_tuning;
BU_HIP_API void bu_hip_get_tuning(const bu_hip_context* , bu_hip_tuning* out, uint32_t struct_bytes);
BU_HIP_API int  bu_hip_set_tuning(bu_hip_context*, const bu_hip_tuning* );

typedef void (*bu_hip_wait_fn)(void* user);
BU_HIP_API int   bu_hip_set_wait_hook(bu_hip_context*, bu_hip_wait_fn fn, void* user);
BU_HIP_API const char* bu_hip_last_error(const bu_hip_context*);

BU_HIP_API int      bu_hip_profile_enable(bu_hip_context*, int on);
BU_HIP_API uint32_t bu_hip_profile_read(bu_hip_context*, const char** names, double* total_ms, uint32_t* launches, uint32_t cap);

BU_HIP_API void* bu_hip_malloc(bu_hip_context*, size_t bytes);
BU_HIP_API void  bu_hip_free(bu_hip_context*, void* d_ptr);
BU_HIP_API int   bu_hip_memcpy_h2d(bu_hip_context*, void* d_dst, const void* h_src, size_t bytes);
BU_HIP_API int bu_hip_memcpy_h2d_async(bu_hip_context*, void* d_dst, const void* h_src, size_t bytes);
BU_HIP_API int   bu_hip_memcpy_d2h(bu_hip_context*, void* h_dst, const void* d_src, size_t bytes);
BU_HIP_API void* bu_hip_host_alloc(size_t bytes);
BU_HIP_API void  bu_hip_host_free(void* p);
typedef struct bu_hip_download bu_hip_download;
BU_HIP_API bu_hip_download* bu_hip_download_begin(bu_hip_context*, void* h_dst, const void* d_src, size_t bytes);
BU_HIP_API int   bu_hip_download_wait(bu_hip_download*);
BU_HIP_API int   bu_hip_memset(bu_hip_context*, void* d_dst, int value, size_t bytes);
BU_HIP_API int   bu_hip_memcpy_d2d(bu_hip_context*, void* d_dst, const void* d_src, size_t bytes);

BU_HIP_API int   bu_hip_set_pixel_blocks_device(bu_hip_context*, size_t total_blocks, const void* d_pixel_blocks);
BU_HIP_API const void* bu_hip_get_pixel_blocks_device(const bu_hip_context*, size_t* total_blocks);

BU_HIP_API int bu_hip_k_extract_blocks(bu_hip_context*, const void* d_rgba, uint32_t width, uint32_t height, uint32_t pitch_bytes, void* d_out_pixel_blocks);

enum { BU_HIP_SLICE_AS_IS = 0, BU_HIP_SLICE_RGB = 1, BU_HIP_SLICE_ALPHA = 2 };
typedef struct bu_hip_slice_source {
    const void* d_raster;
    uint32_t width, height;
    uint32_t pitch_bytes;
    uint32_t mode;
    uint64_t first_block;
} bu_hip_slice_source;
BU_HIP_API int bu_hip_k_extract_slices(bu_hip_context*, const bu_hip_slice_source* slices, uint32_t n, void* d_out_pixel_blocks);

BU_HIP_API int bu_hip_k_prepare_source(bu_hip_context*, const void* d_src, uint32_t width, uint32_t height, uint32_t src_pitch_bytes, void* d_dst, uint32_t dst_pitch_bytes,
        int renormalize, uint32_t swizzle, int check_for_alpha, int force_alpha, int y_flip, uint32_t* out_has_alpha, uint32_t* out_alpha_below_255);
BU_HIP_API int bu_hip_k_renormalize_normal_map(bu_hip_context*, void* d_rgba, uint32_t width, uint32_t height, uint32_t pitch_bytes);
BU_HIP_API int bu_hip_k_split_alpha(bu_hip_context*, const void* d_rgba, uint32_t width, uint32_t height, uint32_t pitch_bytes, void* d_out_rgb, uint32_t rgb_pitch_bytes,
        void* d_out_alpha, uint32_t alpha_pitch_bytes);

enum { BU_ETC_QUALITY_FAST = 0, BU_ETC_QUALITY_MEDIUM = 1, BU_ETC_QUALITY_SLOW = 2, BU_ETC_QUALITY_UBER = 3 };

BU_HIP_API int bu_hip_k_encode_etc1s_blocks(bu_hip_context*, const void* d_pixel_blocks, uint32_t n_blocks, int quality, int perceptual, void* d_out_etc_blocks);
BU_HIP_API int bu_hip_k_upload_and_encode_etc1s_blocks(bu_hip_context*, void* d_pixel_blocks, const void* h_pixel_blocks, uint32_t n_blocks, int quality, int perceptual,
    void* d_out_etc_blocks);
BU_HIP_API int bu_hip_k_endpoint_training_vectors(bu_hip_context*, const void* d_etc_blocks, uint32_t n_blocks, float* d_out_vec6);
BU_HIP_API int bu_hip_k_generate_endpoint_codebook(bu_hip_context*, const void* d_pixel_blocks, uint32_t n_clusters,
    const uint32_t* h_offsets, const uint32_t* d_offsets, const uint32_t* d_indices, int quality, int perceptual, uint32_t step,
    uint8_t* d_params, uint64_t* d_err, uint8_t* d_valid);
BU_HIP_API int bu_hip_k_cluster_colour_means(bu_hip_context*, const void* d_pixel_blocks, uint32_t n_clusters, const uint32_t* h_offsets, const uint32_t* d_indices, float* h_out);
BU_HIP_API int bu_hip_k_refit_endpoints_given_selectors(bu_hip_context*, const void* d_pixel_blocks, const void* d_encoded_blocks, uint32_t n_clusters,
    const uint32_t* h_offsets, const uint32_t* d_offsets, const uint32_t* d_indices, int perceptual,
    uint8_t* d_params, uint64_t* d_err, uint8_t* d_valid, uint64_t* d_current_err);
BU_HIP_API int bu_hip_k_refit_endpoints_given_selectors_q(bu_hip_context*, const void* d_pixel_blocks, const void* d_encoded_blocks, uint32_t n_clusters,
    const uint32_t* h_offsets, const uint32_t* d_offsets, const uint32_t* d_indices, int quality, int perceptual,
    uint8_t* d_params, uint64_t* d_err, uint8_t* d_valid, uint64_t* d_current_err);
BU_HIP_API int bu_hip_k_subblock_errors(bu_hip_context*, const void* d_pixel_blocks, uint32_t n_blocks, const uint32_t* d_block_cluster,
    const uint8_t* d_cluster_params, int perceptual, uint64_t* d_out_err);
BU_HIP_API int bu_hip_k_backend_block_errors(bu_hip_context*, const void* d_pixel_blocks, const void* d_etc_blocks, const uint32_t* d_block_cluster, const uint8_t* d_cluster_params,
    uint32_t first_block, uint32_t num_blocks_x, uint32_t num_blocks_y, uint32_t n_clusters, int perceptual, int with_neighbours, uint32_t* d_own_err, uint32_t* d_neighbour_err);
BU_HIP_API int bu_hip_k_generate_endpoint_codebook_part(bu_hip_context*, const void* d_pixel_blocks, uint32_t n_clusters,
    const uint32_t* h_offsets, const uint32_t* d_offsets, const uint32_t* d_indices, int quality, int perceptual, uint32_t step,
    uint8_t* d_params, uint64_t* d_err, uint8_t* d_valid, uint32_t part, uint32_t parts);
BU_HIP_API int bu_hip_k_refine_endpoint_clusterization(bu_hip_context*, const void* d_pixel_blocks, uint32_t n_blocks,
    const uint32_t* d_block_cluster, const uint8_t* d_cluster_params, uint32_t n_clusters, uint32_t n_parents,
    const uint32_t* d_cand_offsets, const uint32_t* d_cand_indices, const uint8_t* d_block_parent, int perceptual, uint32_t* d_out_best_cluster);
BU_HIP_API int bu_hip_k_resample_rgba8(bu_hip_context*, const void* d_src, uint32_t src_w, uint32_t src_h, void* d_dst, uint32_t dst_w, uint32_t dst_h,
    const uint32_t* x_first, const uint16_t* x_pixel, const float* x_weight, const uint32_t* y_first, const uint16_t* y_pixel, const float* y_weight,
    int x_after_y, int srgb, const float* srgb_to_linear_256, const uint8_t* linear_to_srgb_8192, uint32_t num_comps);
BU_HIP_API int bu_hip_k_determine_selectors(bu_hip_context*, const void* d_pixel_blocks, uint32_t n_blocks,
    const uint8_t* d_color5_inten, const uint32_t* d_block_cluster, int perceptual, void* d_out_etc_blocks);
BU_HIP_API int bu_hip_k_selector_training_vectors(bu_hip_context*, const void* d_encoded_blocks, uint32_t n_blocks, int perceptual, float* d_out_vec16, uint64_t* d_out_weight);
BU_HIP_API int bu_hip_k_create_optimized_selector_codebook(bu_hip_context*, const void* d_pixel_blocks, const void* d_encoded_blocks,
    uint32_t n_clusters, const uint32_t* d_offsets, const uint32_t* d_block_indices, int perceptual, void* d_selector_blocks);
BU_HIP_API int bu_hip_k_find_optimal_selector_clusters(bu_hip_context*, const void* d_pixel_blocks, void* d_encoded_blocks, uint32_t n_blocks,
    const void* d_selector_blocks, uint32_t n_selectors, uint32_t n_parents, const uint32_t* d_cand_offsets, const uint32_t* d_cand_indices,
    const uint8_t* d_block_parent, int perceptual, uint32_t chunk, uint32_t* d_out_block_selector_cluster);

BU_HIP_API int bu_hip_k_encode_uastc_blocks(bu_hip_context*, const void* d_pixel_blocks, uint32_t n_blocks, uint32_t flags, void* d_out_uastc_blocks);
BU_HIP_API size_t bu_hip_uastc_workspace_bytes(uint32_t n_blocks, uint32_t flags);
BU_HIP_API size_t bu_hip_uastc_rdo_workspace_bytes(uint32_t n_blocks, uint32_t total_jobs);

typedef struct bu_uastc_rdo_params {
    float m_lambda;
    float m_max_allowed_rms_increase_ratio;
    float m_skip_block_rms_thresh;
    float m_max_smooth_block_std_dev;
    float m_smooth_block_max_error_scale;
    uint32_t m_lz_dict_size;
    uint32_t m_lz_literal_cost;
    uint32_t m_endpoint_refinement;
} bu_uastc_rdo_params;
BU_HIP_API void bu_hip_uastc_rdo_default_params(bu_uastc_rdo_params* out);
BU_HIP_API int bu_hip_k_uastc_rdo(bu_hip_context*, void* d_uastc_blocks, const void* d_pixel_blocks, uint32_t n_blocks, const bu_uastc_rdo_params* params,
                                  uint32_t flags, uint32_t total_jobs, uint32_t out_stats[4]);
BU_HIP_API int bu_hip_k_uastc_rdo_slices(bu_hip_context*, void* d_uastc_blocks, const void* d_pixel_blocks, const uint32_t* slice_blocks, uint32_t n_slices,
                                         const bu_uastc_rdo_params* params, uint32_t flags, uint32_t total_jobs, uint32_t* out_stats);
BU_HIP_API size_t bu_hip_uastc_rdo_slices_workspace_bytes(const uint32_t* slice_blocks, uint32_t n_slices, uint32_t total_jobs);
BU_HIP_API int bu_hip_uastc_rdo(bu_hip_context*, bu_uastc_block* blocks, const bu_uastc_rdo_params* params, uint32_t flags, uint32_t total_jobs,
                                uint32_t out_stats[4]);

typedef struct bu_uastc_pipeline bu_uastc_pipeline;
BU_HIP_API bu_uastc_pipeline* bu_hip_uastc_pipeline_create(bu_hip_context*, uint32_t lanes, uint32_t max_blocks, uint32_t flags, uint32_t max_total_jobs);
BU_HIP_API int  bu_hip_uastc_pipeline_submit(bu_uastc_pipeline*, const void* d_pixel_blocks, uint32_t n_blocks, void* d_out_uastc_blocks, const bu_uastc_rdo_params* rdo_or_null,
                                             uint32_t flags, uint32_t total_jobs, uint64_t* out_ticket);
BU_HIP_API int  bu_hip_uastc_pipeline_wait(bu_uastc_pipeline*, uint64_t ticket, uint32_t out_stats[4]);
BU_HIP_API void bu_hip_uastc_pipeline_destroy(bu_uastc_pipeline*);

BU_HIP_API int bu_hip_k_transcode_uastc(bu_hip_context*, const void* d_uastc_blocks, uint32_t num_blocks_x, uint32_t num_blocks_y,
        uint32_t orig_width, uint32_t orig_height, uint32_t target, uint32_t decode_flags, int32_t channel0, int32_t channel1,
        void* d_out, uint32_t out_row_pitch_pixels, uint32_t out_rows_pixels, uint32_t* out_invalid_blocks);
BU_HIP_API size_t bu_hip_transcode_output_bytes(uint32_t num_blocks_x, uint32_t num_blocks_y, uint32_t orig_width, uint32_t orig_height, uint32_t target);

BU_HIP_API int bu_hip_k_transcode_etc1s(bu_hip_context*, const void* d_endpoint_palette, uint32_t n_endpoints, const void* d_selector_palette, uint32_t n_selectors,
        const void* d_endpoint_idx, const void* d_selector_idx, const void* d_alpha_endpoint_idx, const void* d_alpha_selector_idx, uint32_t num_blocks_x, uint32_t num_blocks_y,
        uint32_t orig_width, uint32_t orig_height, uint32_t target, void* d_out, uint32_t out_row_pitch_pixels, uint32_t out_rows_pixels);
BU_HIP_API int bu_hip_k_transcode_etc1s_counted(bu_hip_context*, const void* d_endpoint_palette, uint32_t n_endpoints, const void* d_selector_palette, uint32_t n_selectors,
        const void* d_endpoint_idx, const void* d_selector_idx, const void* d_alpha_endpoint_idx, const void* d_alpha_selector_idx, uint32_t num_blocks_x, uint32_t num_blocks_y,
        uint32_t orig_width, uint32_t orig_height, uint32_t target, void* d_out, uint32_t out_row_pitch_pixels, uint32_t out_rows_pixels, uint32_t* out_invalid_blocks);
BU_HIP_API int bu_hip_etc1s_bc1_endpoint_tables(bu_hip_context*, uint32_t* h_out5, uint32_t* h_out6);
BU_HIP_API size_t bu_hip_etc1s_transcode_output_bytes(uint32_t num_blocks_x, uint32_t num_blocks_y, uint32_t orig_width, uint32_t orig_height, uint32_t target,
        uint32_t out_row_pitch_pixels, uint32_t out_rows_pixels);

#define BU_HIP_NO_ALPHA_SLICE UINT64_MAX
typedef struct bu_hip_transcode_slice {
    uint64_t first_block;
    uint64_t alpha_first_block;
    uint64_t out_offset;
    uint32_t num_blocks_x, num_blocks_y;
    uint32_t orig_width, orig_height;
    uint32_t out_row_pitch_pixels, out_rows_pixels;
} bu_hip_transcode_slice;
BU_HIP_API int bu_hip_k_transcode_uastc_slices(bu_hip_context*, const void* d_uastc_blocks, uint64_t n_blocks, const bu_hip_transcode_slice* slices, uint32_t n_slices,
        uint32_t target, uint32_t decode_flags, int32_t channel0, int32_t channel1, void* d_out, size_t out_bytes, uint32_t* out_invalid_per_slice);
BU_HIP_API int bu_hip_k_transcode_etc1s_slices(bu_hip_context*, const void* d_endpoint_palette, uint32_t n_endpoints, const void* d_selector_palette, uint32_t n_selectors,
        const void* d_endpoint_idx, const void* d_selector_idx, uint64_t n_indices, const bu_hip_transcode_slice* slices, uint32_t n_slices, uint32_t target,
        void* d_out, size_t out_bytes, uint32_t* out_invalid_per_slice);
BU_HIP_API size_t bu_hip_transcode_slice_extent(const bu_hip_transcode_slice*, uint32_t target, int etc1s);

BU_HIP_API int bu_hip_k_unpack_blocks(bu_hip_context*, const void* d_blocks, uint32_t num_blocks_x, uint32_t num_blocks_y,
        uint32_t orig_width, uint32_t orig_height, uint32_t format, void* d_out_rgba, uint32_t out_row_pitch_pixels,
        uint32_t out_rows_pixels, uint32_t* out_invalid_blocks);
BU_HIP_API size_t bu_hip_unpack_output_bytes(uint32_t num_blocks_x, uint32_t num_blocks_y, uint32_t orig_width, uint32_t orig_height,
        uint32_t out_row_pitch_pixels, uint32_t out_rows_pixels);

enum { BU_HIP_DDS_BC1 = 0, BU_HIP_DDS_BC2 = 1, BU_HIP_DDS_BC3 = 2, BU_HIP_DDS_BC4 = 3, BU_HIP_DDS_BC5 = 4, BU_HIP_DDS_BC7 = 5, BU_HIP_DDS_A8R8G8B8 = 6,
       BU_HIP_DDS_A8B8G8R8 = 7, BU_HIP_DDS_R8 = 8, BU_HIP_DDS_R8G8 = 9, BU_HIP_DDS_R5G6B5 = 10, BU_HIP_DDS_A1R5G5B5 = 11, BU_HIP_DDS_A4R4G4B4 = 12 };
BU_HIP_API int bu_hip_k_pack_dds_blocks(bu_hip_context*, const void* d_tiles, uint64_t n_tiles, uint32_t format, void* d_out);
BU_HIP_API int bu_hip_k_pack_dds_pixels(bu_hip_context*, const void* d_tiles, uint64_t n_tiles, const bu_hip_transcode_slice* slices, uint32_t n_slices, uint32_t format,
        void* d_out, size_t out_bytes);
BU_HIP_API size_t bu_hip_dds_payload_bytes(const bu_hip_transcode_slice* slices, uint32_t n_slices, uint32_t format);

typedef struct bu_image_metrics_counts {
    uint32_t struct_bytes;
    uint32_t width, height;
    uint32_t reserved;
    uint32_t hist[6][256];
    uint64_t sum_a[4], sum_b[4];
} bu_image_metrics_counts;
BU_HIP_API int bu_hip_k_image_metrics(bu_hip_context*, const void* d_a, uint32_t width_a, uint32_t height_a, uint32_t pitch_a_pixels, const void* d_b, uint32_t width_b,
        uint32_t height_b, uint32_t pitch_b_pixels, bu_image_metrics_counts* h_out);

typedef struct bu_psnr_hvs_sums {
    uint32_t struct_bytes;
    uint32_t width, height;
    uint32_t blocks;
    double sum_hvs[6], sum_hvsm[6];
} bu_psnr_hvs_sums;
BU_HIP_API int bu_hip_k_psnr_hvs(bu_hip_context*, const void* d_a, uint32_t width_a, uint32_t height_a, uint32_t pitch_a_pixels, const void* d_b, uint32_t width_b,
        uint32_t height_b, uint32_t pitch_b_pixels, bu_psnr_hvs_sums* h_out);
BU_HIP_API int bu_hip_k_psnr_hvs_blocks(bu_hip_context*, const void* d_a, uint32_t width_a, uint32_t height_a, uint32_t pitch_a_pixels, const void* d_b, uint32_t width_b,
        uint32_t height_b, uint32_t pitch_b_pixels, uint32_t mode, double* h_out_blocks, uint32_t capacity_blocks, uint32_t* out_blocks);

typedef struct bu_ssim_result {
    uint32_t struct_bytes;
    uint32_t width, height;
    uint32_t chunks_walked;
    float r, g, b, rgb, a, luma_709, luma_601;
    uint32_t chunks;
} bu_ssim_result;
BU_HIP_API int bu_hip_k_ssim(bu_hip_context*, const void* d_a, uint32_t width_a, uint32_t height_a, uint32_t pitch_a_pixels, const void* d_b, uint32_t width_b,
        uint32_t height_b, uint32_t pitch_b_pixels, bu_ssim_result* h_out);
BU_HIP_API int bu_hip_k_ssim_map(bu_hip_context*, const void* d_a, uint32_t width_a, uint32_t height_a, uint32_t pitch_a_pixels, const void* d_b, uint32_t width_b,
        uint32_t height_b, uint32_t pitch_b_pixels, uint32_t mode, float* h_out, uint64_t capacity_floats, uint32_t* out_pixels);

BU_HIP_API int bu_hip_k_map_blocks_from_groups(bu_hip_context*, const uint32_t* d_group_offsets, const uint32_t* d_sorted_block_idx, uint32_t n_blocks, uint32_t u_total,
    const uint32_t* d_leaf_of_unique, const uint32_t* d_first_pos, const uint32_t* d_parent_of_unique, uint32_t* d_out_cluster, uint32_t* d_out_pos, uint8_t* d_out_parent);
BU_HIP_API int bu_hip_k_map_rank_blocks(bu_hip_context*, const uint32_t* d_block_cluster, uint32_t n_blocks, uint32_t n_clusters, uint32_t* d_out_sizes,
    uint32_t* d_out_offsets, uint32_t* d_out_sorted_blocks, uint32_t* d_out_pos);
BU_HIP_API int bu_hip_k_map_endpoint_csr(bu_hip_context*, const uint32_t* d_block_cluster, const uint32_t* d_block_pos, uint32_t n_blocks, const uint32_t* d_offsets,
    uint32_t* d_out_indices);
BU_HIP_API int bu_hip_k_map_remap(bu_hip_context*, uint32_t* d_block_cluster, uint32_t* d_block_pos, uint32_t n_blocks, const uint32_t* d_new_index, const uint32_t* d_base);
BU_HIP_API int bu_hip_k_map_count_differences(bu_hip_context*, const uint32_t* d_a, const uint32_t* d_b, uint32_t n, uint32_t* d_out_count);
BU_HIP_API int bu_hip_k_map_membership(bu_hip_context*, const uint8_t* d_block_parent, const uint32_t* d_block_cluster, uint32_t n_blocks, uint32_t n_parents,
    uint32_t n_clusters, uint8_t* d_out_flags);
BU_HIP_API int bu_hip_k_map_gather(bu_hip_context*, const uint32_t* d_table, const uint32_t* d_index, uint32_t n, uint32_t* d_out);

BU_HIP_API int bu_hip_kmeans_codebook(bu_hip_context*, int kind, const void* d_keys, const uint64_t* d_weights, const uint32_t* d_group_offsets, uint32_t n_vectors,
    uint32_t max_clusters, uint32_t n_parents, uint32_t iterations, uint32_t* d_out_cluster_of_vector, uint32_t* d_out_parent_of_vector, uint32_t* out_clusters,
    uint32_t* out_parents);
BU_HIP_API int bu_hip_k_kmeans_seed(bu_hip_context*, int kind, const void* d_keys, const uint64_t* d_weights, const uint32_t* d_group_offsets, uint32_t n_vectors, uint32_t k,
    uint32_t* d_out_pick, float* d_out_centroids);
BU_HIP_API int bu_hip_k_kmeans_round(bu_hip_context*, int kind, const void* d_keys, const uint64_t* d_weights, const uint32_t* d_group_offsets, uint32_t n_vectors, uint32_t k,
    float* d_centroids, uint64_t* d_live, int update, uint32_t* d_out_assign, uint64_t* d_out_sums, uint64_t* d_out_worst);

typedef struct bu_tsvq bu_tsvq;
#define BU_TSVQ_BUFFERS 4u
typedef struct { float origin[16]; uint64_t weight; float var; uint32_t pad; } bu_tsvq_root;
typedef struct { uint32_t buf, start, count, pad; uint64_t weight; float origin[16]; } bu_tsvq_node;
typedef struct { uint32_t ok, l_count, r_count, pad; uint64_t l_weight, r_weight; float l_var, r_var; float l_centroid[16], r_centroid[16]; } bu_tsvq_split;
BU_HIP_API bu_tsvq* bu_hip_tsvq_create(bu_hip_context*, uint32_t dim, const float* h_rows, const uint64_t* h_weights, uint32_t n, bu_tsvq_root* h_out_root);
BU_HIP_API bu_tsvq* bu_hip_tsvq_create_packed16(bu_hip_context*, const uint32_t* h_keys, const uint64_t* h_weights, uint32_t n, bu_tsvq_root* h_out_root);
BU_HIP_API bu_tsvq* bu_hip_tsvq_create_packed16_device(bu_hip_context*, const uint32_t* d_keys, const uint64_t* d_weights, uint32_t n, bu_tsvq_root* h_out_root);
BU_HIP_API bu_tsvq* bu_hip_tsvq_create_endpoint_device(bu_hip_context*, const uint64_t* d_unique_keys, const uint32_t* d_group_offsets, uint32_t n, bu_tsvq_root* h_out_root);
BU_HIP_API int bu_hip_k_unique_endpoint_vectors(bu_hip_context*, const void* d_etc1_blocks, uint32_t n_blocks, uint32_t* d_sorted_block_idx, uint64_t* d_unique_keys,
                                                uint32_t* d_group_offsets, uint32_t* out_unique);
BU_HIP_API int bu_hip_k_unique_selector_vectors(bu_hip_context*, const void* d_enc_blocks, const uint64_t* d_weights, uint32_t n_blocks, uint32_t* d_sorted_block_idx,
                                                uint32_t* d_unique_keys, uint64_t* d_unique_weights, uint32_t* d_group_offsets, uint32_t* out_unique);
BU_HIP_API int  bu_hip_tsvq_split(bu_hip_context*, bu_tsvq*, const bu_tsvq_node* h_nodes, uint32_t n_nodes, bu_tsvq_split* h_out);
BU_HIP_API int  bu_hip_tsvq_split_deep(bu_hip_context*, bu_tsvq*, const bu_tsvq_node* h_nodes, uint32_t n_nodes, bu_tsvq_split* h_out, uint32_t levels, bu_tsvq_split* h_deep);
BU_HIP_API int  bu_hip_tsvq_roots(bu_hip_context*, bu_tsvq*, const bu_tsvq_node* h_nodes, uint32_t n_nodes, bu_tsvq_root* h_out);
BU_HIP_API int  bu_hip_tsvq_read_members(bu_hip_context*, bu_tsvq*, uint32_t buf, uint32_t start, uint32_t count, uint32_t* h_out);
typedef struct { uint32_t buf, start, count, value; } bu_tsvq_span;
BU_HIP_API int  bu_hip_tsvq_scatter_spans(bu_hip_context*, bu_tsvq*, const bu_tsvq_span* h_spans, uint32_t n_spans, uint32_t* d_out);
BU_HIP_API int  bu_hip_tsvq_finish_spans(bu_hip_context*, bu_tsvq*, const bu_tsvq_span* h_spans, uint32_t n_spans, uint32_t* d_leaf_of, uint32_t* d_parent_of,
                                         const uint32_t* d_group_offsets, uint32_t* d_first_pos, uint32_t* d_sizes);
BU_HIP_API int  bu_hip_tsvq_exchange_pack(bu_hip_context*, bu_tsvq*, const bu_tsvq_node* h_nodes, const uint8_t* h_mine, const bu_tsvq_split* h_records, uint32_t n_nodes,
                                          void** d_staging, uint64_t* n_u64);
BU_HIP_API int  bu_hip_tsvq_exchange_unpack(bu_hip_context*, bu_tsvq*, const bu_tsvq_node* h_nodes, const uint8_t* h_mine, bu_tsvq_split* h_records, uint32_t n_nodes);
BU_HIP_API void bu_hip_tsvq_destroy(bu_hip_context*, bu_tsvq*);

#ifdef __cplusplus
}
#endif
#endif
```

Baseline: 1239 Mpixels/s.

## Replace rocprim/hipcub sort and run-length passes with custom LSD radix sort

Adds a hand-written tile-based LSD radix sort for u32 key/value pairs, with up to 9-bit digits, per-tile histograms, a row scan and a wave-ballot stable scatter. It replaces the rocprim sort_pairs and the hipcub RLE, scan and ReduceByKey passes in cluster ranking and in unique endpoint/selector extraction. The value array is implicit (iota) when null, which drops the iota copy kernel. Offsets and sizes are now computed in one kernel, and run emission uses custom head-count and emit kernels. The aim is fewer launches and less traffic, but the custom sort may be slower than the tuned library sort for 32-bit keys, which need four passes.

```diff
diff --git a/basis_universal_amd/csrc/api_etc1s.cpp b/basis_universal_amd/csrc/api_etc1s.cpp
--- a/basis_universal_amd/csrc/api_etc1s.cpp
+++ b/basis_universal_amd/csrc/api_etc1s.cpp
@@ -5,6 +5,7 @@
 #include "mipmap_kernels.h"
 #include "unique_kernels.h"
 #include "bookkeeping_kernels.h"
+#include "radix_pairs.h"
 #include "kmeans_kernels.h"
 #include "host/seam_translate.h"
 
@@ -442,7 +443,22 @@
     return 1;
 }
 
-int bu_hip_k_map_endpoint_csr(bu_hip_context* ctx, const uint32_t* d_cluster, const uint32_t* d_pos, uint32_t n, const uint32_t* d_offsets, uint32_t* d_indices) {
+int bu_hip_k_sort_pairs_u32(bu_hip_context* ctx, const uint32_t* d_keys, const uint32_t* d_values, uint32_t n, uint32_t begin_bit, uint32_t end_bit, uint32_t* d_keys_out,
+                            uint32_t* d_values_out) {
+    if (!ctx) return 0;
+    if (!d_keys || !d_keys_out || !d_values_out) { set_error(ctx, "sort_pairs_u32: null pointer"); return 0; }
+    if (begin_bit >= end_bit || end_bit > 32) { set_error(ctx, "sort_pairs_u32: need begin_bit < end_bit <= 32"); return 0; }
+    if (d_keys_out == d_keys || (d_values && d_values_out == d_values)) { set_error(ctx, "sort_pairs_u32: the outputs must not be the inputs"); return 0; }
+    if (n > bu::RADIX_MAX_ITEMS) { set_error(ctx, "sort_pairs_u32: too many items"); return 0; }
+    if (!n) return 1;
+    device_guard g(ctx->device);
+    arena& ws = ctx->scratch[4];
+    BU_TRY(ctx, ws.reserve(bu::radix_pairs_workspace_bytes(n, begin_bit, end_bit)));
+    BU_TRY(ctx, bu::radix_sort_pairs(ctx->stream, ws.p, d_keys, d_values, n, begin_bit, end_bit, d_keys_out, d_values_out));
+    return 1;
+}
+
+int bu_hip_k_map_endpoint_csr(bu_hip_context* ctx,const uint32_t* d_cluster, const uint32_t* d_pos, uint32_t n, const uint32_t* d_offsets, uint32_t* d_indices) {
     if (!ctx) return 0;
     device_guard g(ctx->device);
     prof_scope ps(ctx, "map_endpoint_csr");
diff --git a/basis_universal_amd/csrc/bookkeeping_kernels.hip b/basis_universal_amd/csrc/bookkeeping_kernels.hip
--- a/basis_universal_amd/csrc/bookkeeping_kernels.hip
+++ b/basis_universal_amd/csrc/bookkeeping_kernels.hip
@@ -1,10 +1,9 @@
 #include <hip/hip_runtime.h>
-#include <hipcub/hipcub.hpp>
 #include <stdint.h>
 #include <algorithm>
 
 #include "bookkeeping_kernels.h"
-#include "sort_pairs.h"
+#include "radix_pairs.h"
 #include "tsvq_bufs.h"
 
 namespace bu {
@@ -25,20 +24,18 @@
     if (parent) parent[b] = parent_of_unique ? (uint8_t)parent_of_unique[u] : 0;
 }
 
-__global__ void __launch_bounds__(256) k_iota_copy(const uint32_t* __restrict__ src, uint32_t n, uint32_t* __restrict__ keys, uint32_t* __restrict__ vals) {
-    const uint32_t i = blockIdx.x * 256 + threadIdx.x;
-    if (i < n) { keys[i] = src[i]; vals[i] = i; }
-}
-__global__ void __launch_bounds__(256) k_offsets_from_sorted(const uint32_t* __restrict__ keys_sorted, uint32_t n, uint32_t k, uint32_t* __restrict__ offsets) {
+__device__ inline uint32_t first_not_below(const uint32_t* __restrict__ keys_sorted, uint32_t n, uint32_t c) {
+    uint32_t lo = 0, hi = n;
+    while (lo < hi) { const uint32_t mid = (lo + hi) >> 1; if (keys_sorted[mid] < c) lo = mid + 1; else hi = mid; }
+    return lo;
+}
+__global__ void __launch_bounds__(256) k_offsets_sizes_from_sorted(const uint32_t* __restrict__ keys_sorted, uint32_t n, uint32_t k, uint32_t* __restrict__ offsets,
+                                                                   uint32_t* __restrict__ sizes) {
     const uint32_t c = blockIdx.x * 256 + threadIdx.x;
     if (c > k) return;
-    uint32_t lo = 0, hi = n;
-    while (lo < hi) { const uint32_t mid = (lo + hi) >> 1; if (keys_sorted[mid] < c) lo = mid + 1; else hi = mid; }
-    offsets[c] = lo;
-}
-__global__ void __launch_bounds__(256) k_sizes_from_offsets(const uint32_t* __restrict__ offsets, uint32_t k, uint32_t* __restrict__ sizes) {
-    const uint32_t c = blockIdx.x * 256 + threadIdx.x;
-    if (c <= k) sizes[c] = c < k ? offsets[c + 1] - offsets[c] : 0u;
+    const uint32_t at = first_not_below(keys_sorted, n, c);
+    offsets[c] = at;
+    sizes[c] = c < k ? first_not_below(keys_sorted, n, c + 1) - at : 0u;
 }
 __global__ void __launch_bounds__(256) k_positions(const uint32_t* __restrict__ keys_sorted, const uint32_t* __restrict__ blocks_sorted, uint32_t n,
                                                    const uint32_t* __restrict__ offsets, uint32_t* __restrict__ pos) {
@@ -143,20 +140,20 @@
     if (i < n) out[i] = table[index[i]];
 }
 
-struct rank_temp { uint32_t *keys_in, *vals_in, *keys_sorted; void* cub; size_t cub_bytes; };
-
+struct rank_temp { uint32_t* keys_sorted; void* sort; };
+
+unsigned cluster_bits(uint32_t k) {
+    unsigned bits = 1;
+    while (bits < 32 && (1u << bits) < k) bits++;
+    return bits;
+}
 rank_temp carve_rank(void* ws, uint32_t n, uint32_t k, size_t* total) {
     auto up = [](size_t x) { return (x + 255) & ~(size_t)255; };
-    size_t sort_bytes = 0, scan_bytes = 0;
-    (void)sort_pairs<uint32_t, uint32_t>(nullptr, sort_bytes, nullptr, nullptr, nullptr, nullptr, n, 0, 32, nullptr);
-    (void)hipcub::DeviceScan::ExclusiveSum(nullptr, scan_bytes, (const uint32_t*)nullptr, (uint32_t*)nullptr, (int)k + 1);
     rank_temp t;
     char* p = static_cast<char*>(ws);
     size_t off = 0;
-    t.keys_in = reinterpret_cast<uint32_t*>(p + off); off += up((size_t)n * 4);
-    t.vals_in = reinterpret_cast<uint32_t*>(p + off); off += up((size_t)n * 4);
     t.keys_sorted = reinterpret_cast<uint32_t*>(p + off); off += up((size_t)n * 4);
-    t.cub = p + off; t.cub_bytes = up(sort_bytes > scan_bytes ? sort_bytes : scan_bytes); off += t.cub_bytes;
+    t.sort = p + off; off += up(radix_pairs_workspace_bytes(n, 0, cluster_bits(k)));
     if (total) *total = off;
     return t;
 }
@@ -179,13 +176,8 @@
     const rank_temp t = carve_rank(d_ws, n, k, nullptr);
     hipError_t e;
     const dim3 grid((n + 255) / 256), blk(256), gk((k + 256) / 256);
-    hipLaunchKernelGGL(k_iota_copy, grid, blk, 0, st, d_cluster, n, t.keys_in, t.vals_in);
-    int bits = 1;
-    while (bits < 32 && (1u << bits) < k) bits++;
-    size_t bytes = t.cub_bytes;
-    if ((e = sort_pairs<uint32_t, uint32_t>(t.cub, bytes, t.keys_in, t.keys_sorted, t.vals_in, d_sorted_blocks, n, 0, (unsigned)bits, st)) != hipSuccess) return e;
-    hipLaunchKernelGGL(k_offsets_from_sorted, gk, blk, 0, st, t.keys_sorted, n, k, d_offsets);
-    hipLaunchKernelGGL(k_sizes_from_offsets, gk, blk, 0, st, d_offsets, k, d_sizes);
+    if ((e = radix_sort_pairs(st, t.sort, d_cluster, nullptr, n, 0, cluster_bits(k), t.keys_sorted, d_sorted_blocks)) != hipSuccess) return e;
+    hipLaunchKernelGGL(k_offsets_sizes_from_sorted, gk, blk, 0, st, t.keys_sorted, n, k, d_offsets, d_sizes);
     if (d_pos) hipLaunchKernelGGL(k_positions, grid, blk, 0, st, t.keys_sorted, d_sorted_blocks, n, d_offsets, d_pos);
     return hipGetLastError();
 }
diff --git a/basis_universal_amd/csrc/radix_pairs.h b/basis_universal_amd/csrc/radix_pairs.h
--- /dev/null
+++ b/basis_universal_amd/csrc/radix_pairs.h
@@ -0,0 +1,19 @@
+#pragma once
+#include <hip/hip_runtime.h>
+#include <stdint.h>
+
+namespace bu {
+
+constexpr uint32_t RADIX_TILE = 2048;
+constexpr uint32_t RADIX_MAX_DIGIT_BITS = 9;
+constexpr uint32_t RADIX_MAX_ITEMS = 0x7FFFF800u;
+
+inline uint32_t radix_tiles(uint32_t n) { return (uint32_t)(((uint64_t)n + RADIX_TILE - 1) / RADIX_TILE); }
+
+size_t radix_pairs_workspace_bytes(uint32_t n, unsigned begin_bit, unsigned end_bit);
+hipError_t radix_sort_pairs(hipStream_t st, void* d_workspace, const uint32_t* d_keys_in, const uint32_t* d_values_in, uint32_t n, unsigned begin_bit, unsigned end_bit,
+                            uint32_t* d_keys_out, uint32_t* d_values_out);
+
+hipError_t launch_row_scan(hipStream_t st, uint32_t* d_matrix, uint32_t rows, uint32_t cols, uint32_t* d_totals);
+
+}
diff --git a/basis_universal_amd/csrc/radix_pairs_kernels.hip b/basis_universal_amd/csrc/radix_pairs_kernels.hip
--- /dev/null
+++ b/basis_universal_amd/csrc/radix_pairs_kernels.hip
@@ -0,0 +1,186 @@
+#include <hip/hip_runtime.h>
+#include <stdint.h>
+
+#include "radix_pairs.h"
+
+namespace bu {
+
+namespace {
+
+constexpr uint32_t THREADS = 256, WAVES = 4, ROUNDS = RADIX_TILE / THREADS, MAX_BINS = 1u << RADIX_MAX_DIGIT_BITS;
+static_assert(ROUNDS * THREADS == RADIX_TILE && MAX_BINS == 2 * THREADS, "the digit scan below gives every thread two bins");
+
+__device__ inline uint32_t block_exclusive_sum(uint32_t v, uint32_t* s_wave, uint32_t* total) {
+    const uint32_t lane = threadIdx.x & 63, wave = threadIdx.x >> 6;
+    uint32_t incl = v;
+#pragma unroll
+    for (uint32_t o = 1; o < 64; o <<= 1) { const uint32_t t = (uint32_t)__shfl_up((int)incl, o, 64); if (lane >= o) incl += t; }
+    __syncthreads();
+    if (lane == 63) s_wave[wave] = incl;
+    __syncthreads();
+    uint32_t before = 0;
+    for (uint32_t w = 0; w < wave; w++) before += s_wave[w];
+    *total = s_wave[0] + s_wave[1] + s_wave[2] + s_wave[3];
+    return before + incl - v;
+}
+
+__global__ void __launch_bounds__(256) k_digit_counts(const uint32_t* __restrict__ keys, uint32_t n, uint32_t shift, uint32_t bits, uint32_t tiles, uint32_t* __restrict__ counts) {
+    __shared__ uint32_t s_hist[MAX_BINS];
+    const uint32_t bins = 1u << bits, mask = bins - 1;
+    s_hist[threadIdx.x] = 0; s_hist[threadIdx.x + THREADS] = 0;
+    __syncthreads();
+    const uint32_t base = blockIdx.x * RADIX_TILE;
+#pragma unroll
+    for (uint32_t r = 0; r < ROUNDS; r++) {
+        const uint32_t i = base + r * THREADS + threadIdx.x;
+        if (i < n) atomicAdd(&s_hist[(keys[i] >> shift) & mask], 1u);
+    }
+    __syncthreads();
+    for (uint32_t d = threadIdx.x; d < bins; d += THREADS) counts[(size_t)d * tiles + blockIdx.x] = s_hist[d];
+}
+
+__global__ void __launch_bounds__(256) k_row_scan(uint32_t* __restrict__ matrix, uint32_t cols, uint32_t* __restrict__ totals) {
+    __shared__ uint32_t s_wave[WAVES];
+    uint32_t* row = matrix + (size_t)blockIdx.x * cols;
+    uint32_t run = 0;
+    for (uint32_t base = 0; base < cols; base += 4 * THREADS) {
+        const uint32_t i0 = base + threadIdx.x * 4;
+        uint32_t v[4], mine = 0;
+#pragma unroll
+        for (uint32_t j = 0; j < 4; j++) { v[j] = i0 + j < cols ? row[i0 + j] : 0u; mine += v[j]; }
+        uint32_t total;
+        uint32_t at = run + block_exclusive_sum(mine, s_wave, &total);
+#pragma unroll
+        for (uint32_t j = 0; j < 4; j++) { if (i0 + j < cols) row[i0 + j] = at; at += v[j]; }
+        run += total;
+    }
+    if (threadIdx.x == 0) totals[blockIdx.x] = run;
+}
+
+__global__ void __launch_bounds__(256) k_scatter(const uint32_t* __restrict__ keys_in, const uint32_t* __restrict__ values_in , uint32_t n, uint32_t shift,
+                                                 uint32_t bits, uint32_t tiles, const uint32_t* __restrict__ counts , const uint32_t* __restrict__ totals,
+                                                 uint32_t* __restrict__ keys_out, uint32_t* __restrict__ values_out) {
+    __shared__ uint32_t s_cnt[WAVES][MAX_BINS];
+    __shared__ uint32_t s_out[MAX_BINS];
+    __shared__ uint32_t s_keys[RADIX_TILE], s_vals[RADIX_TILE];
+    __shared__ uint32_t s_wave[WAVES];
+    const uint32_t bins = 1u << bits, mask = bins - 1;
+    const uint32_t lane = threadIdx.x & 63, wave = threadIdx.x >> 6;
+    for (uint32_t j = threadIdx.x; j < WAVES * MAX_BINS; j += THREADS) (&s_cnt[0][0])[j] = 0;
+    __syncthreads();
+
+    const uint32_t base = blockIdx.x * RADIX_TILE, in_tile = n - base < RADIX_TILE ? n - base : RADIX_TILE;
+    uint32_t key[ROUNDS], rank[ROUNDS];
+#pragma unroll
+    for (uint32_t r = 0; r < ROUNDS; r++) {
+        const uint32_t i = base + wave * (ROUNDS * 64) + r * 64 + lane;
+        key[r] = i < n ? keys_in[i] : 0xFFFFFFFFu;
+        const uint32_t d = i < n ? (key[r] >> shift) & mask : mask;
+        uint64_t same = ~0ull;
+        for (uint32_t b = 0; b < bits; b++) {
+            const bool one = (d >> b) & 1u;
+            const uint64_t vote = __ballot(one);
+            same &= one ? vote : ~vote;
+        }
+        const uint32_t before = (uint32_t)__popcll(same & ((1ull << lane) - 1ull));
+        const uint32_t seen = s_cnt[wave][d];
+        rank[r] = seen + before;
+        __syncthreads();
+        if (before == 0) s_cnt[wave][d] = seen + (uint32_t)__popcll(same);
+        __syncthreads();
+    }
+
+    const uint32_t d0 = threadIdx.x * 2;
+    uint32_t c[2][WAVES], local[2] = { 0, 0 }, global[2];
+#pragma unroll
+    for (uint32_t e = 0; e < 2; e++) {
+#pragma unroll
+        for (uint32_t w = 0; w < WAVES; w++) { c[e][w] = s_cnt[w][d0 + e]; local[e] += c[e][w]; }
+        global[e] = d0 + e < bins ? totals[d0 + e] : 0u;
+    }
+    uint32_t unused;
+    const uint32_t local_at = block_exclusive_sum(local[0] + local[1], s_wave, &unused);
+    const uint32_t global_at = block_exclusive_sum(global[0] + global[1], s_wave, &unused);
+#pragma unroll
+    for (uint32_t e = 0; e < 2; e++) {
+        uint32_t at = local_at + (e ? local[0] : 0u);
+        if (d0 + e < bins) s_out[d0 + e] = global_at + (e ? global[0] : 0u) + counts[(size_t)(d0 + e) * tiles + blockIdx.x] - at;
+#pragma unroll
+        for (uint32_t w = 0; w < WAVES; w++) { s_cnt[w][d0 + e] = at; at += c[e][w]; }
+    }
+    __syncthreads();
+
+#pragma unroll
+    for (uint32_t r = 0; r < ROUNDS; r++) {
+        const uint32_t i = base + wave * (ROUNDS * 64) + r * 64 + lane;
+        const uint32_t d = i < n ? (key[r] >> shift) & mask : mask;
+        const uint32_t at = s_cnt[wave][d] + rank[r];
+        s_keys[at] = key[r];
+        s_vals[at] = i < n ? (values_in ? values_in[i] : i) : 0u;
+    }
+    __syncthreads();
+#pragma unroll
+    for (uint32_t r = 0; r < ROUNDS; r++) {
+        const uint32_t j = r * THREADS + threadIdx.x;
+        if (j < in_tile) {
+            const uint32_t k = s_keys[j];
+            const uint32_t to = s_out[(k >> shift) & mask] + j;
+            keys_out[to] = k;
+            values_out[to] = s_vals[j];
+        }
+    }
+}
+
+struct pass_plan { uint32_t passes, width; };
+pass_plan plan_for(unsigned begin_bit, unsigned end_bit) {
+    const uint32_t total = end_bit - begin_bit;
+    pass_plan p;
+    p.passes = (total + RADIX_MAX_DIGIT_BITS - 1) / RADIX_MAX_DIGIT_BITS;
+    p.width = (total + p.passes - 1) / p.passes;
+    return p;
+}
+size_t up256(size_t v) { return (v + 255) & ~(size_t)255; }
+
+}
+
+size_t radix_pairs_workspace_bytes(uint32_t n, unsigned begin_bit, unsigned end_bit) {
+    if (begin_bit >= end_bit || end_bit > 32) return 0;
+    const pass_plan p = plan_for(begin_bit, end_bit);
+    const size_t matrix = up256(((size_t)1 << p.width) * radix_tiles(n ? n : 1) * 4) + up256(MAX_BINS * 4);
+    return matrix + (p.passes > 1 ? 2 * up256((size_t)(n ? n : 1) * 4) : 0);
+}
+
+hipError_t launch_row_scan(hipStream_t st, uint32_t* d_matrix, uint32_t rows, uint32_t cols, uint32_t* d_totals) {
+    if (!rows) return hipSuccess;
+    hipLaunchKernelGGL(k_row_scan, dim3(rows), dim3(THREADS), 0, st, d_matrix, cols, d_totals);
+    return hipGetLastError();
+}
+
+hipError_t radix_sort_pairs(hipStream_t st, void* d_workspace, const uint32_t* d_keys_in, const uint32_t* d_values_in, uint32_t n, unsigned begin_bit, unsigned end_bit,
+                            uint32_t* d_keys_out, uint32_t* d_values_out) {
+    if (begin_bit >= end_bit || end_bit > 32 || n > RADIX_MAX_ITEMS) return hipErrorInvalidValue;
+    if (!n) return hipSuccess;
+    const pass_plan p = plan_for(begin_bit, end_bit);
+    const uint32_t tiles = radix_tiles(n);
+    char* ws = static_cast<char*>(d_workspace);
+    uint32_t* counts = reinterpret_cast<uint32_t*>(ws);
+    uint32_t* totals = reinterpret_cast<uint32_t*>(ws + up256(((size_t)1 << p.width) * tiles * 4));
+    uint32_t* keys_tmp = totals + up256(MAX_BINS * 4) / 4;
+    uint32_t* vals_tmp = keys_tmp + up256((size_t)n * 4) / 4;
+    const uint32_t* keys = d_keys_in;
+    const uint32_t* vals = d_values_in;
+    for (uint32_t pass = 0; pass < p.passes; pass++) {
+        const uint32_t shift = begin_bit + pass * p.width;
+        const uint32_t bits = shift + p.width <= end_bit ? p.width : end_bit - shift;
+        const bool to_out = ((p.passes - 1 - pass) & 1u) == 0;
+        uint32_t* ko = to_out ? d_keys_out : keys_tmp;
+        uint32_t* vo = to_out ? d_values_out : vals_tmp;
+        hipLaunchKernelGGL(k_digit_counts, dim3(tiles), dim3(THREADS), 0, st, keys, n, shift, bits, tiles, counts);
+        hipLaunchKernelGGL(k_row_scan, dim3(1u << bits), dim3(THREADS), 0, st, counts, tiles, totals);
+        hipLaunchKernelGGL(k_scatter, dim3(tiles), dim3(THREADS), 0, st, keys, vals, n, shift, bits, tiles, counts, totals, ko, vo);
+        keys = ko; vals = vo;
+    }
+    return hipGetLastError();
+}
+
+}
diff --git a/basis_universal_amd/csrc/sort_pairs.h b/basis_universal_amd/csrc/sort_pairs.h
--- a/basis_universal_amd/csrc/sort_pairs.h
+++ /dev/null
@@ -1,15 +0,0 @@
-#pragma once
-#include <hip/hip_runtime.h>
-#include <rocprim/rocprim.hpp>
-
-namespace bu {
-
-using sort_pairs_config = rocprim::radix_sort_config<rocprim::default_config, rocprim::default_config, rocprim::default_config, 32768>;
-
-template <class Key, class Value>
-inline hipError_t sort_pairs(void* temporary, size_t& bytes, const Key* keys_in, Key* keys_out, const Value* values_in, Value* values_out, size_t n, unsigned begin_bit, unsigned end_bit,
-                             hipStream_t stream) {
-    return rocprim::radix_sort_pairs<sort_pairs_config>(temporary, bytes, keys_in, keys_out, values_in, values_out, n, begin_bit, end_bit, stream);
-}
-
-}
diff --git a/basis_universal_amd/csrc/unique_kernels.hip b/basis_universal_amd/csrc/unique_kernels.hip
--- a/basis_universal_amd/csrc/unique_kernels.hip
+++ b/basis_universal_amd/csrc/unique_kernels.hip
@@ -1,5 +1,4 @@
 #include <hip/hip_runtime.h>
-#include <hipcub/hipcub.hpp>
 #include <stdint.h>
 
 #include <algorithm>
@@ -7,13 +6,13 @@
 #include <vector>
 
 #include "unique_kernels.h"
-#include "sort_pairs.h"
+#include "radix_pairs.h"
 
 namespace bu {
 
 namespace {
 
-__global__ void __launch_bounds__(256) k_selector_keys(const uint64_t* __restrict__ enc_blocks, uint32_t n, uint32_t* __restrict__ keys, uint32_t* __restrict__ idx) {
+__global__ void __launch_bounds__(256) k_selector_keys(const uint64_t* __restrict__ enc_blocks, uint32_t n, uint32_t* __restrict__ keys) {
     const uint32_t b = blockIdx.x * 256 + threadIdx.x;
     if (b >= n) return;
     const uint32_t lo = (uint32_t)__builtin_bswap64(enc_blocks[b]);
@@ -25,16 +24,123 @@
         key = (key << 2) | ((0x1Eu >> (raw * 2u)) & 3u);
     }
     keys[b] = key;
-    idx[b] = b;
-}
-
-__global__ void __launch_bounds__(256) k_close_offsets(const uint32_t* __restrict__ n_runs, uint32_t n, uint32_t* __restrict__ offsets) {
-    if (blockIdx.x == 0 && threadIdx.x == 0) offsets[*n_runs] = n;
-}
-
-__global__ void __launch_bounds__(256) k_gather_weights(const uint32_t* __restrict__ idx, const uint64_t* __restrict__ weights, uint32_t n, uint64_t* __restrict__ out) {
-    const uint32_t j = blockIdx.x * 256 + threadIdx.x;
-    if (j < n) out[j] = weights[idx[j]];
+}
+
+constexpr uint32_t TILE = RADIX_TILE, PER_THREAD = TILE / 256;
+
+__device__ inline uint64_t block_sum_u64(uint64_t v, uint64_t* s_part ) {
+#pragma unroll
+    for (int o = 32; o >= 1; o >>= 1) v += (uint64_t)__shfl_xor((unsigned long long)v, o, 64);
+    __syncthreads();
+    if ((threadIdx.x & 63) == 0) s_part[threadIdx.x >> 6] = v;
+    __syncthreads();
+    return s_part[0] + s_part[1] + s_part[2] + s_part[3];
+}
+
+template <bool WEIGHTS>
+__global__ void __launch_bounds__(256) k_head_counts(const uint32_t* __restrict__ keys, const uint32_t* __restrict__ idx, const uint64_t* __restrict__ weights, uint32_t n,
+                                                     uint32_t* __restrict__ head_counts, uint64_t* __restrict__ lead_sums) {
+    __shared__ uint32_t s_heads, s_first;
+    __shared__ uint64_t s_part[4];
+    if (threadIdx.x == 0) { s_heads = 0; s_first = TILE; }
+    __syncthreads();
+    const uint32_t base = blockIdx.x * TILE;
+    uint32_t heads = 0, first = TILE;
+#pragma unroll
+    for (uint32_t r = 0; r < PER_THREAD; r++) {
+        const uint32_t j = r * 256 + threadIdx.x, i = base + j;
+        if (i < n && (i == 0 || keys[i] != keys[i - 1])) { heads++; if (first == TILE) first = j; }
+    }
+    if (heads) { atomicAdd(&s_heads, heads); if (WEIGHTS) atomicMin(&s_first, first); }
+    __syncthreads();
+    if (threadIdx.x == 0) head_counts[blockIdx.x] = s_heads;
+    if (!WEIGHTS) return;
+    const uint32_t lead = s_first;
+    uint64_t sum = 0;
+#pragma unroll
+    for (uint32_t r = 0; r < PER_THREAD; r++) {
+        const uint32_t j = r * 256 + threadIdx.x, i = base + j;
+        if (i < n && j < lead) sum += weights[idx[i]];
+    }
+    sum = block_sum_u64(sum, s_part);
+    if (threadIdx.x == 0) lead_sums[blockIdx.x] = sum;
+}
+
+template <bool SELECTOR>
+__global__ void __launch_bounds__(256) k_emit_runs(const uint32_t* __restrict__ keys, const uint32_t* __restrict__ idx, const uint64_t* __restrict__ weights, uint32_t n, uint32_t tiles,
+                                                   const uint32_t* __restrict__ heads_before, const uint64_t* __restrict__ lead_sums, const uint64_t* __restrict__ key_of_rank,
+                                                   void* __restrict__ unique_keys, uint64_t* __restrict__ unique_weights, uint32_t* __restrict__ offsets) {
+    __shared__ uint32_t s_key[TILE];
+    __shared__ uint32_t s_head[TILE + 1];
+    __shared__ uint64_t s_sum[SELECTOR ? TILE + 1 : 1];
+    __shared__ uint64_t s_part[4];
+    __shared__ uint32_t s_wave[4];
+    const uint32_t base = blockIdx.x * TILE, in_tile = n - base < TILE ? n - base : TILE;
+#pragma unroll
+    for (uint32_t r = 0; r < PER_THREAD; r++) {
+        const uint32_t j = r * 256 + threadIdx.x;
+        s_key[j] = j < in_tile ? keys[base + j] : 0u;
+        if (SELECTOR) s_sum[j] = j < in_tile ? weights[idx[base + j]] : 0ull;
+    }
+    const bool first_is_head = base == 0 || keys[base] != keys[base - 1];
+    __syncthreads();
+
+    const uint32_t j0 = threadIdx.x * PER_THREAD;
+    uint32_t flags = 0;
+    uint64_t mine = 0;
+#pragma unroll
+    for (uint32_t e = 0; e < PER_THREAD; e++) {
+        const uint32_t j = j0 + e;
+        if (j < in_tile && (j == 0 ? first_is_head : s_key[j] != s_key[j - 1])) flags |= 1u << e;
+        if (SELECTOR) mine += s_sum[j];
+    }
+    const uint32_t lane = threadIdx.x & 63, wave = threadIdx.x >> 6;
+    uint32_t h_incl = (uint32_t)__popc(flags);
+    uint64_t w_incl = mine;
+#pragma unroll
+    for (uint32_t o = 1; o < 64; o <<= 1) {
+        const uint32_t th = (uint32_t)__shfl_up((int)h_incl, o, 64);
+        const uint64_t tw = SELECTOR ? (uint64_t)__shfl_up((unsigned long long)w_incl, o, 64) : 0ull;
+        if (lane >= o) { h_incl += th; w_incl += tw; }
+    }
+    if (lane == 63) { s_wave[wave] = h_incl; s_part[wave] = w_incl; }
+    __syncthreads();
+    uint32_t h_at = h_incl - (uint32_t)__popc(flags), heads = 0;
+    uint64_t w_at = w_incl - mine;
+#pragma unroll
+    for (uint32_t w = 0; w < 4; w++) {
+        if (w < wave) { h_at += s_wave[w]; w_at += s_part[w]; }
+        heads += s_wave[w];
+    }
+#pragma unroll
+    for (uint32_t e = 0; e < PER_THREAD; e++) {
+        const uint32_t j = j0 + e;
+        if (flags & (1u << e)) s_head[h_at++] = j;
+        if (SELECTOR) { const uint64_t w = s_sum[j]; s_sum[j] = w_at; w_at += w; }
+    }
+    if (threadIdx.x == 255) { s_head[heads] = in_tile; if (SELECTOR) s_sum[TILE] = w_at; }
+    __syncthreads();
+
+    const uint32_t u0 = heads_before[blockIdx.x];
+    if (blockIdx.x == tiles - 1 && threadIdx.x == 0) offsets[u0 + heads] = n;
+    if (!heads) return;
+    uint64_t follow = 0;
+    if (SELECTOR) {
+        const uint32_t through = u0 + heads;
+        uint64_t f = 0;
+        for (uint32_t t = blockIdx.x + 1 + threadIdx.x; t < tiles && heads_before[t] == through; t += 256) f += lead_sums[t];
+        follow = block_sum_u64(f, s_part);
+    }
+    for (uint32_t r = threadIdx.x; r < heads; r += 256) {
+        const uint32_t j = s_head[r], end = s_head[r + 1], u = u0 + r;
+        offsets[u] = base + j;
+        if (SELECTOR) {
+            static_cast<uint32_t*>(unique_keys)[u] = s_key[j];
+            unique_weights[u] = s_sum[end == in_tile ? TILE : end] - s_sum[j] + (r == heads - 1 ? follow : 0ull);
+        } else {
+            static_cast<uint64_t*>(unique_keys)[u] = key_of_rank[s_key[j]];
+        }
+    }
 }
 
 __host__ __device__ inline uint64_t endpoint_key_of_code(uint32_t code) {
@@ -75,90 +181,57 @@
 }
 
 __global__ void __launch_bounds__(256) k_endpoint_ranks(const uint64_t* __restrict__ etc1_blocks, uint32_t n, const uint32_t* __restrict__ rank_of_code,
-                                                        uint32_t* __restrict__ ranks, uint32_t* __restrict__ idx) {
+                                                        uint32_t* __restrict__ ranks) {
     const uint32_t b = blockIdx.x * 256 + threadIdx.x;
     if (b >= n) return;
     const uint64_t v = __builtin_bswap64(etc1_blocks[b]);
     const uint32_t code = (uint32_t)(((v >> 59) & 31) << 13 | ((v >> 51) & 31) << 8 | ((v >> 43) & 31) << 3 | ((v >> 37) & 7));
     ranks[b] = rank_of_code[code];
-    idx[b] = b;
-}
-__global__ void __launch_bounds__(256) k_keys_of_ranks(const uint32_t* __restrict__ ranks, const uint32_t* __restrict__ n_runs, const uint64_t* __restrict__ key_of_rank,
-                                                       uint32_t n, uint64_t* __restrict__ keys) {
-    const uint32_t u = blockIdx.x * 256 + threadIdx.x;
-    if (u < n && u < *n_runs) keys[u] = key_of_rank[ranks[u]];
-}
-
-struct unique_temp { uint32_t *keys_in, *idx_in, *keys_sorted, *counts, *n_runs, *keys_again; uint64_t* w_sorted; void* cub; size_t cub_bytes; };
+}
+
+struct unique_temp { uint32_t *keys_in, *keys_sorted, *head_counts, *n_runs; uint64_t* lead_sums; void* sort; };
 size_t align_up(size_t v) { return (v + 255) & ~(size_t)255; }
 
-size_t cub_bytes_for(uint32_t n) {
-    size_t a = 0, b = 0, c = 0, d = 0;
-    uint32_t* p = nullptr;
-    uint64_t* w = nullptr;
-    (void)sort_pairs<uint32_t, uint32_t>(nullptr, a, p, p, p, p, n, 0, 32, nullptr);
-    (void)hipcub::DeviceRunLengthEncode::Encode(nullptr, b, p, p, p, p, (int)n);
-    (void)hipcub::DeviceScan::ExclusiveSum(nullptr, c, p, p, (int)n);
-    (void)hipcub::DeviceReduce::ReduceByKey(nullptr, d, p, p, w, w, p, hipcub::Sum(), (int)n);
-    return std::max(std::max(a, b), std::max(c, d));
-}
-
-unique_temp carve(void* base, uint32_t n, size_t* total) {
+unique_temp carve(void* base, uint32_t n, unsigned key_bits, size_t* total) {
     char* p = static_cast<char*>(base);
     size_t o = 0;
     unique_temp t;
+    const uint32_t tiles = radix_tiles(n);
     t.keys_in = reinterpret_cast<uint32_t*>(p + o); o += align_up((size_t)n * 4);
-    t.idx_in = reinterpret_cast<uint32_t*>(p + o); o += align_up((size_t)n * 4);
     t.keys_sorted = reinterpret_cast<uint32_t*>(p + o); o += align_up((size_t)n * 4);
-    t.counts = reinterpret_cast<uint32_t*>(p + o); o += align_up((size_t)n * 4);
+    t.head_counts = reinterpret_cast<uint32_t*>(p + o); o += align_up((size_t)tiles * 4);
+    t.lead_sums = reinterpret_cast<uint64_t*>(p + o); o += align_up((size_t)tiles * 8);
     t.n_runs = reinterpret_cast<uint32_t*>(p + o); o += 256;
-    t.keys_again = reinterpret_cast<uint32_t*>(p + o); o += align_up((size_t)n * 4);
-    t.w_sorted = reinterpret_cast<uint64_t*>(p + o); o += align_up((size_t)n * 8);
-    t.cub_bytes = cub_bytes_for(n);
-    t.cub = p + o; o += align_up(t.cub_bytes);
+    t.sort = p + o; o += align_up(radix_pairs_workspace_bytes(n, 0, key_bits));
     if (total) *total = o;
     return t;
 }
 
-struct unique64_temp { uint64_t *keys_in, *keys_sorted; uint32_t *idx_in, *counts, *n_runs; void* cub; size_t cub_bytes; };
-size_t cub_bytes_for64(uint32_t n) {
-    size_t a = 0, b = 0, c = 0;
-    uint64_t* k = nullptr;
-    uint32_t* p = nullptr;
-    (void)sort_pairs<uint64_t, uint32_t>(nullptr, a, k, k, p, p, n, 0, 64, nullptr);
-    (void)hipcub::DeviceRunLengthEncode::Encode(nullptr, b, k, k, p, p, (int)n);
-    (void)hipcub::DeviceScan::ExclusiveSum(nullptr, c, p, p, (int)n);
-    size_t a32 = 0, b32 = 0;
-    (void)sort_pairs<uint32_t, uint32_t>(nullptr, a32, p, p, p, p, n, 0, 18, nullptr);
-    (void)hipcub::DeviceRunLengthEncode::Encode(nullptr, b32, p, p, p, p, (int)n);
-    return std::max(std::max(a, a32), std::max(std::max(b, b32), c));
-}
-unique64_temp carve64(void* base, uint32_t n, size_t* total) {
-    char* p = static_cast<char*>(base);
-    size_t o = 0;
-    unique64_temp t;
-    t.keys_in = reinterpret_cast<uint64_t*>(p + o); o += align_up((size_t)n * 8);
-    t.keys_sorted = reinterpret_cast<uint64_t*>(p + o); o += align_up((size_t)n * 8);
-    t.idx_in = reinterpret_cast<uint32_t*>(p + o); o += align_up((size_t)n * 4);
-    t.counts = reinterpret_cast<uint32_t*>(p + o); o += align_up((size_t)n * 4);
-    t.n_runs = reinterpret_cast<uint32_t*>(p + o); o += 256;
-    t.cub_bytes = cub_bytes_for64(n);
-    t.cub = p + o; o += align_up(t.cub_bytes);
-    if (total) *total = o;
-    return t;
+constexpr unsigned ENDPOINT_RANK_BITS = 18, SELECTOR_KEY_BITS = 32;
+
+template <bool SELECTOR>
+hipError_t emit_runs(hipStream_t st, const unique_temp& t, const uint32_t* d_sorted_block_idx, const uint64_t* d_weights, uint32_t n, const uint64_t* key_of_rank, void* d_unique_keys,
+                     uint64_t* d_unique_weights, uint32_t* d_group_offsets) {
+    const uint32_t tiles = radix_tiles(n);
+    hipLaunchKernelGGL(k_head_counts<SELECTOR>, dim3(tiles), dim3(256), 0, st, t.keys_sorted, d_sorted_block_idx, d_weights, n, t.head_counts, t.lead_sums);
+    const hipError_t e = launch_row_scan(st, t.head_counts, 1, tiles, t.n_runs);
+    if (e != hipSuccess) return e;
+    hipLaunchKernelGGL(k_emit_runs<SELECTOR>, dim3(tiles), dim3(256), 0, st, t.keys_sorted, d_sorted_block_idx, d_weights, n, tiles, t.head_counts, t.lead_sums, key_of_rank,
+                       d_unique_keys, d_unique_weights, d_group_offsets);
+    return hipGetLastError();
 }
 
 }
 
 size_t unique_endpoint_vectors_workspace_bytes(uint32_t n_blocks) {
     size_t total = 0;
-    carve64(nullptr, n_blocks ? n_blocks : 1, &total);
+    carve(nullptr, n_blocks ? n_blocks : 1, ENDPOINT_RANK_BITS, &total);
     return total;
 }
 
 hipError_t launch_unique_endpoint_vectors(hipStream_t st, const void* d_etc1_blocks, uint32_t n, void* d_workspace, uint32_t* d_sorted_block_idx, uint64_t* d_unique_keys,
                                           uint32_t* d_group_offsets, uint32_t** d_n_unique) {
-    const unique64_temp t = carve64(d_workspace, n, nullptr);
+    const unique_temp t = carve(d_workspace, n ? n : 1, ENDPOINT_RANK_BITS, nullptr);
     if (d_n_unique) *d_n_unique = t.n_runs;
     if (!n) return hipMemsetAsync(t.n_runs, 0, 4, st);
     int device = 0;
@@ -166,52 +239,27 @@
     if (e != hipSuccess) return e;
     const endpoint_rank_tables& tab = endpoint_tables(device);
     if (tab.status != hipSuccess) return tab.status;
-    uint32_t* ranks_in = reinterpret_cast<uint32_t*>(t.keys_in);
-    uint32_t* ranks_sorted = ranks_in + n;
-    uint32_t* ranks_unique = reinterpret_cast<uint32_t*>(t.keys_sorted);
-    hipLaunchKernelGGL(k_endpoint_ranks, dim3((n + 255) / 256), dim3(256), 0, st, static_cast<const uint64_t*>(d_etc1_blocks), n, tab.rank_of_code, ranks_in, t.idx_in);
-    size_t bytes = t.cub_bytes;
-    e = sort_pairs<uint32_t, uint32_t>(t.cub, bytes, ranks_in, ranks_sorted, t.idx_in, d_sorted_block_idx, n, 0, 18, st);
-    if (e != hipSuccess) return e;
-    bytes = t.cub_bytes;
-    e = hipcub::DeviceRunLengthEncode::Encode(t.cub, bytes, ranks_sorted, ranks_unique, t.counts, t.n_runs, (int)n, st);
-    if (e != hipSuccess) return e;
-    bytes = t.cub_bytes;
-    e = hipcub::DeviceScan::ExclusiveSum(t.cub, bytes, t.counts, d_group_offsets, (int)n, st);
-    if (e != hipSuccess) return e;
-    hipLaunchKernelGGL(k_close_offsets, dim3(1), dim3(64), 0, st, t.n_runs, n, d_group_offsets);
-    const uint32_t most = n < tab.n_ranks ? n : tab.n_ranks;
-    hipLaunchKernelGGL(k_keys_of_ranks, dim3((most + 255) / 256), dim3(256), 0, st, ranks_unique, t.n_runs, tab.key_of_rank, most, d_unique_keys);
-    return hipGetLastError();
+    hipLaunchKernelGGL(k_endpoint_ranks, dim3((n + 255) / 256), dim3(256), 0, st, static_cast<const uint64_t*>(d_etc1_blocks), n, tab.rank_of_code, t.keys_in);
+    e = radix_sort_pairs(st, t.sort, t.keys_in, nullptr, n, 0, ENDPOINT_RANK_BITS, t.keys_sorted, d_sorted_block_idx);
+    if (e != hipSuccess) return e;
+    return emit_runs<false>(st, t, d_sorted_block_idx, nullptr, n, tab.key_of_rank, d_unique_keys, nullptr, d_group_offsets);
 }
 
 size_t unique_selector_vectors_workspace_bytes(uint32_t n_blocks) {
     size_t total = 0;
-    carve(nullptr, n_blocks ? n_blocks : 1, &total);
+    carve(nullptr, n_blocks ? n_blocks : 1, SELECTOR_KEY_BITS, &total);
     return total;
 }
 
 hipError_t launch_unique_selector_vectors(hipStream_t st, const void* d_enc_blocks, const uint64_t* d_weights, uint32_t n, void* d_workspace, uint32_t* d_sorted_block_idx,
                                           uint32_t* d_unique_keys, uint64_t* d_unique_weights, uint32_t* d_group_offsets, uint32_t** d_n_unique) {
-    const unique_temp t = carve(d_workspace, n, nullptr);
+    const unique_temp t = carve(d_workspace, n ? n : 1, SELECTOR_KEY_BITS, nullptr);
     if (d_n_unique) *d_n_unique = t.n_runs;
     if (!n) return hipMemsetAsync(t.n_runs, 0, 4, st);
-    hipLaunchKernelGGL(k_selector_keys, dim3((n + 255) / 256), dim3(256), 0, st, static_cast<const uint64_t*>(d_enc_blocks), n, t.keys_in, t.idx_in);
-    size_t bytes = t.cub_bytes;
-    hipError_t e = sort_pairs<uint32_t, uint32_t>(t.cub, bytes, t.keys_in, t.keys_sorted, t.idx_in, d_sorted_block_idx, n, 0, 32, st);
-    if (e != hipSuccess) return e;
-    bytes = t.cub_bytes;
-    e = hipcub::DeviceRunLengthEncode::Encode(t.cub, bytes, t.keys_sorted, d_unique_keys, t.counts, t.n_runs, (int)n, st);
-    if (e != hipSuccess) return e;
-    bytes = t.cub_bytes;
-    e = hipcub::DeviceScan::ExclusiveSum(t.cub, bytes, t.counts, d_group_offsets, (int)n, st);
-    if (e != hipSuccess) return e;
-    hipLaunchKernelGGL(k_close_offsets, dim3(1), dim3(64), 0, st, t.n_runs, n, d_group_offsets);
-    hipLaunchKernelGGL(k_gather_weights, dim3((n + 255) / 256), dim3(256), 0, st, d_sorted_block_idx, d_weights, n, t.w_sorted);
-    bytes = t.cub_bytes;
-    e = hipcub::DeviceReduce::ReduceByKey(t.cub, bytes, t.keys_sorted, t.keys_again, t.w_sorted, d_unique_weights, t.n_runs + 1, hipcub::Sum(), (int)n, st);
-    if (e != hipSuccess) return e;
-    return hipGetLastError();
-}
-
-}
+    hipLaunchKernelGGL(k_selector_keys, dim3((n + 255) / 256), dim3(256), 0, st, static_cast<const uint64_t*>(d_enc_blocks), n, t.keys_in);
+    const hipError_t e = radix_sort_pairs(st, t.sort, t.keys_in, nullptr, n, 0, SELECTOR_KEY_BITS, t.keys_sorted, d_sorted_block_idx);
+    if (e != hipSuccess) return e;
+    return emit_runs<true>(st, t, d_sorted_block_idx, d_weights, n, nullptr, d_unique_keys, d_unique_weights, d_group_offsets);
+}
+
+}
diff --git a/include/basisu_hip.h b/include/basisu_hip.h
--- a/include/basisu_hip.h
+++ b/include/basisu_hip.h
@@ -275,6 +275,8 @@
 BU_HIP_API int bu_hip_k_map_membership(bu_hip_context*, const uint8_t* d_block_parent, const uint32_t* d_block_cluster, uint32_t n_blocks, uint32_t n_parents,
     uint32_t n_clusters, uint8_t* d_out_flags);
 BU_HIP_API int bu_hip_k_map_gather(bu_hip_context*, const uint32_t* d_table, const uint32_t* d_index, uint32_t n, uint32_t* d_out);
+BU_HIP_API int bu_hip_k_sort_pairs_u32(bu_hip_context*, const uint32_t* d_keys, const uint32_t* d_values, uint32_t n, uint32_t begin_bit, uint32_t end_bit,
+    uint32_t* d_keys_out, uint32_t* d_values_out);
 
 BU_HIP_API int bu_hip_kmeans_codebook(bu_hip_context*, int kind, const void* d_keys, const uint64_t* d_weights, const uint32_t* d_group_offsets, uint32_t n_vectors,
     uint32_t max_clusters, uint32_t n_parents, uint32_t iterations, uint32_t* d_out_cluster_of_vector, uint32_t* d_out_parent_of_vector, uint32_t* out_clusters,
```

Result: no change. 1253 Mpixels/s (median of 4 runs) (+1.1%).
